# kessel/dune-pnp

Measured on AMD Instinct MI355X. Metric: assembled DOFs/s + BiCGStab iters/s, 3-species PNP on pore.msh-refined, higher is better.
Workload: dtype f64; 1 GPU; config 3: stationary 3-ion PNP, test/pore_pnp/pore.msh refined k=4 x 1 mirrored copies; dofs=2214099, dofs_per_gpu=2214099, mesh_vertices=738033, triangles=1470464, parallelism=mesh partition (RCB) x1, preconditioner=ilu0, colors=4, sell_slots=5176768, blocks=5155025

## Files before the change

### dune-pnp_amd/csrc/assemble.hip

```cpp
#include <cstdlib>

#include <hip/hip_ext.h>

#include "element.h"
#include "kernels.h"

namespace pnp {

namespace {

template <int OP, int KC = 0>
__device__ __forceinline__ void store_block(double *__restrict__ vc, int lane, int s,
                                            const double *Kc) {
  constexpr int NK = OpTraits<OP>::NK;
  static_assert(!KC || OP == OP_PNP, "constant planes: the PNP operator only");
  constexpr int Q0 = KC ? 2 : 0;
#ifdef ASM_STORE_PLAIN
  store_vals<NK, Q0>(vc + size_t(s) * NK * kRows, lane, Kc);
#else
  store_vals_nt<NK, Q0>(vc + size_t(s) * NK * kRows, lane, Kc);
#endif
}

template <int OP, int JAC, int MINW, int FANR>
__global__ __launch_bounds__(256, MINW) void k_assemble(DevLayout L, AsmArgs a) {
  using T = OpTraits<OP>;
  constexpr int NF = T::NF, NK = T::NK;
  const int row = xcd_block(blockIdx.x, gridDim.x, L.xcd_remap) * blockDim.x + threadIdx.x;
  if (row >= L.n_owned) return;
  const int chunk = row / kRows, lane = row % kRows;
  const int off = L.chunk_off[chunk];
  const uint64_t meta = L.rowmeta[row];
  const int len = int(meta & 63);
  const bool closed = (meta >> 6) & 1;
  const unsigned brk = unsigned(meta >> 8);
  const int *__restrict__ cix = L.colidx + off + lane;
  double *__restrict__ vc = a.vals + size_t(off) * NK;

  const double2 pi2 = reinterpret_cast<const double2 *>(L.xy)[row];
  double ui[NF];
#pragma unroll
  for (int f = 0; f < NF; f++) ui[f] = a.x[size_t(row) * NF + f];
  double ai = 0, aq = 0;
  if constexpr (OP == OP_DIFF || OP == OP_DIFF_IE || OP == OP_POISSON) ai = a.aux0[row];
  if constexpr (OP == OP_POISSON) aq = a.aux1[row];
  if constexpr (OP == OP_PB) pb_fifth(ui[0], ai, aq);

  double R[NF], D[NK], P[NK], F[NK];
#pragma unroll
  for (int f = 0; f < NF; f++) R[f] = 0;
#pragma unroll
  for (int v = 0; v < NK; v++) D[v] = P[v] = F[v] = 0;

  auto next_slot = [&](int s) { return (s + 1 < len) ? s + 1 : (closed ? 1 : -1); };
  auto load_nb = [&](int j, double2 &p, double (&u)[NF], double &a0, double &a1) {
    p = reinterpret_cast<const double2 *>(L.xy)[j];
    load_nf<NF>(a.x, size_t(j), u);
    if constexpr (OP == OP_DIFF || OP == OP_DIFF_IE || OP == OP_POISSON) a0 = a.aux0[j];
    if constexpr (OP == OP_POISSON) a1 = a.aux1[j];
  };
  double2 pc, pn;
  double uc[NF], un[NF];
  double ac0 = 0, ac1 = 0, an0 = 0, an1 = 0;
  constexpr int NC = FANR > 0 ? FANR : 1;
  int cj[NC];
  if constexpr (FANR > 0) {
#pragma unroll
    for (int k = 1; k < FANR; k++) cj[k] = cix[(k < len ? k : 0) * kRows];
  }
  auto col = [&](int k) -> int {
    if constexpr (FANR > 0)
      return cj[k];
    else
      return cix[k * kRows];
  };
  load_nb(col(1), pc, uc, ac0, ac1);
  if constexpr (OP == OP_PB) pb_fifth(uc[0], ac0, ac1);
  {
    const int t1 = next_slot(1);
    if (t1 > 0) load_nb(t1 == 1 ? col(1) : col(2), pn, un, an0, an1);
  }
  int jn = -1;
  if constexpr (FANR == 0) {
    const int t2 = next_slot(1) > 0 ? next_slot(next_slot(1)) : -1;
    if (t2 > 0 && next_slot(1) != 1) jn = cix[t2 * kRows];
  }
  for (int s = 1; s < len; ++s) {
    const int t = next_slot(s);
    const int tn = (t > 0 && t != 1) ? next_slot(t) : -1;
    double2 pp = pn;
    double up[NF];
    double ap0 = 0, ap1 = 0;
    if (tn > 0) {
      if constexpr (FANR > 0) {
        load_nb(tn == 1 ? col(1) : col(s + 2), pp, up, ap0, ap1);
      } else {
        load_nb(jn, pp, up, ap0, ap1);
        const int tnn = tn != 1 ? next_slot(tn) : -1;
        jn = tnn > 0 ? cix[tnn * kRows] : -1;
      }
    }
    const bool elem = t > 0 && !((brk >> s) & 1);
    if constexpr (OP == OP_PB)
      if (t > 0) pb_fifth(un[0], an0, an1);
    if (elem) {
      Geo G;
      geometry(pi2.x, pi2.y, pc.x, pc.y, pn.x, pn.y, G);
      double Ct[NK];
#pragma unroll
      for (int v = 0; v < NK; v++) Ct[v] = 0;
      element<OP, JAC>(a, G, pi2.y, pc.y, pn.y, ui, uc, un, ai, ac0, an0, aq, ac1, an1, R, D, P,
                       Ct);
      if constexpr (JAC) {
        if (s == 1 && closed) {
#pragma unroll
          for (int v = 0; v < NK; v++) F[v] = P[v];
        } else {
          store_block<OP>(vc, lane, s, P);
        }
#pragma unroll
        for (int v = 0; v < NK; v++) P[v] = Ct[v];
      }
    } else if constexpr (JAC) {
      store_block<OP>(vc, lane, s, P);
#pragma unroll
      for (int v = 0; v < NK; v++) P[v] = 0;
    }
    pc = pn;
#pragma unroll
    for (int f = 0; f < NF; f++) uc[f] = un[f];
    ac0 = an0;
    ac1 = an1;
    if (tn > 0) {
      pn = pp;
#pragma unroll
      for (int f = 0; f < NF; f++) un[f] = up[f];
      an0 = ap0;
      an1 = ap1;
    }
  }
  if constexpr (JAC) {
    if (closed) {
#pragma unroll
      for (int v = 0; v < NK; v++) F[v] += P[v];
      store_block<OP>(vc, lane, 1, F);
    }
    store_block<OP>(vc, lane, 0, D);
  }
#pragma unroll
  for (int f = 0; f < NF; f++) {
    const size_t q = size_t(row) * NF + f;
    const double rv = R[f] + a.cvec[q];
    a.r[q] = a.dmask[q] != 0 ? 0.0 : rv;
  }
}

#ifndef ASM_SU
#define ASM_SU 4
#endif
template <int OP>
__host__ __device__ constexpr int asm_lds_rec() {
  return 2 + OpTraits<OP>::NF + (OP == OP_DIFF || OP == OP_DIFF_IE || OP == OP_POISSON) +
         (OP == OP_POISSON);
}
template <int OP>
constexpr int asm_kc() {
  return OP == OP_PNP;
}
template <int OP, int JAC, int MINW, int FANR, int SPLIT = FANR, int STAGE = 0, int LDSG = 0,
          int KC = 0>
__global__ __launch_bounds__(256, MINW) void k_assemble_ga(DevLayout L, AsmArgs a) {
  using T = OpTraits<OP>;
  constexpr int NF = T::NF, NK = T::NK, NS = FANR;
  constexpr bool AUX0 = OP == OP_DIFF || OP == OP_DIFF_IE || OP == OP_POISSON;
  constexpr bool AUX1 = OP == OP_POISSON;
  constexpr int RW = asm_lds_rec<OP>();
  extern __shared__ double srec[];
  const int blk = row_block(L, blockIdx.x, gridDim.x);
  const int row0 = blk * blockDim.x + threadIdx.x;
  const bool live = row0 < L.n_owned;
  if (!LDSG && !live) return;
  const int row = live ? row0 : 0;
  const int chunk = row / kRows, lane = row % kRows;
  const int off = L.chunk_off[chunk];
  const uint64_t meta = L.rowmeta[row];
  const int len = int(meta & 63);
  const bool closed = (meta >> 6) & 1;
  const unsigned brk = unsigned(meta >> 8);
  double *__restrict__ vc = a.vals + size_t(off) * NK;

  int cj[NS];
  if constexpr (LDSG) {
    const uint16_t *__restrict__ lix = L.lidx + off + lane;
#pragma unroll
    for (int k = 1; k < NS; k++) {
      const int t = lix[(k < len ? k : 0) * kRows];
      cj[k] = k < len ? t : 0;
    }
  } else {
    const int *__restrict__ cix = L.colidx + off + lane;
#pragma unroll
    for (int k = 1; k < NS; k++) cj[k] = cix[(k < len ? k : 0) * kRows];
  }
  const double2 pi2 = reinterpret_cast<const double2 *>(L.xy)[row];
  double ui[NF];
  load_nf<NF>(a.x, size_t(row), ui);
  double ai = 0, aq = 0;
  if constexpr (AUX0) ai = a.aux0[row];
  if constexpr (AUX1) aq = a.aux1[row];
  if constexpr (OP == OP_PB) pb_fifth(ui[0], ai, aq);
  if constexpr (LDSG) {
    const int u0 = L.uptr[blk], cnt = L.uown[blk];
    constexpr int kSU = ASM_SU;
    int jj[kSU];
#pragma unroll
    for (int u = 0; u < kSU; u++) {
      const int k = int(threadIdx.x) + u * 256;
      jj[u] = k < cnt ? L.ulist[u0 + k] : -1;
    }
    double t[kSU][RW];
#pragma unroll
    for (int u = 0; u < kSU; u++)
      if (jj[u] >= 0) {
        const double2 p = reinterpret_cast<const double2 *>(L.xy)[jj[u]];
        t[u][0] = p.x;
        t[u][1] = p.y;
        double uu[NF];
        load_nf<NF>(a.x, size_t(jj[u]), uu);
#pragma unroll
        for (int f = 0; f < NF; f++) t[u][2 + f] = uu[f];
        if constexpr (AUX0) t[u][2 + NF] = a.aux0[jj[u]];
        if constexpr (AUX1) t[u][3 + NF] = a.aux1[jj[u]];
      }
#pragma unroll
    for (int u = 0; u < kSU; u++)
      if (jj[u] >= 0)
#pragma unroll
        for (int w = 0; w < RW; w++) srec[size_t(int(threadIdx.x) + u * 256) * RW + w] = t[u][w];
    for (int k = int(threadIdx.x) + kSU * 256; k < cnt; k += blockDim.x) {
      const int j = L.ulist[u0 + k];
      const double2 p = reinterpret_cast<const double2 *>(L.xy)[j];
      double u[NF];
      load_nf<NF>(a.x, size_t(j), u);
      double *r = srec + size_t(k) * RW;
      r[0] = p.x;
      r[1] = p.y;
#pragma unroll
      for (int f = 0; f < NF; f++) r[2 + f] = u[f];
      if constexpr (AUX0) r[2 + NF] = a.aux0[j];
      if constexpr (AUX1) r[3 + NF] = a.aux1[j];
    }
    __syncthreads();
    if (!live) return;
  }
  double2 pn[NS];
  double un[NS][NF], a0[NS], a1[NS];
  auto gather = [&](int k) {
    if constexpr (LDSG) {
      const double *r = srec + size_t(cj[k]) * RW;
      pn[k] = make_double2(r[0], r[1]);
#pragma unroll
      for (int f = 0; f < NF; f++) un[k][f] = r[2 + f];
      a0[k] = AUX0 ? r[2 + NF] : 0.0;
      a1[k] = AUX1 ? r[3 + NF] : 0.0;
    } else {
      pn[k] = reinterpret_cast<const double2 *>(L.xy)[cj[k]];
      load_nf<NF>(a.x, size_t(cj[k]), un[k]);
      a0[k] = AUX0 ? a.aux0[cj[k]] : 0.0;
      a1[k] = AUX1 ? a.aux1[cj[k]] : 0.0;
    }
  };
#pragma unroll
  for (int k = 1; k < SPLIT; k++) gather(k);
  if constexpr (OP == OP_PB) pb_fifth(un[1][0], a0[1], a1[1]);

  double R[NF], D[NK], P[NK], F[NK];
#pragma unroll
  for (int f = 0; f < NF; f++) R[f] = 0;
#pragma unroll
  for (int v = 0; v < NK; v++) D[v] = P[v] = F[v] = 0;
  constexpr int NSTG = (STAGE && JAC && SPLIT < NS && SPLIT > 3) ? SPLIT - 3 : 0;
  __shared__ double stg[NSTG > 0 ? NSTG * NK * 256 : 1];
  unsigned staged = 0;
  auto put = [&](int s, const double *Kc) {
    if (NSTG > 0 && s <= NSTG) {
#pragma unroll
      for (int v = 0; v < NK; v++) stg[((s - 1) * NK + v) * 256 + threadIdx.x] = Kc[v];
      staged |= 1u << s;
    } else {
      store_block<OP, KC>(vc, lane, s, Kc);
    }
  };
#pragma unroll
  for (int s = 1; s < NS; s++) {
    if (SPLIT < NS && s == (SPLIT > 2 ? SPLIT - 2 : 1)) {
#pragma unroll
      for (int k = SPLIT; k < NS; k++) gather(k);
      if constexpr (NSTG > 0) {
#pragma unroll
        for (int q = 1; q <= NSTG; q++)
          if ((staged >> q) & 1) {
            double K[NK];
#pragma unroll
            for (int v = 0; v < NK; v++) K[v] = stg[((q - 1) * NK + v) * 256 + threadIdx.x];
            store_block<OP, KC>(vc, lane, q, K);
          }
      }
    }
    if (s < len) {
      const bool has_next = s + 1 < len;
      const int sn = (s + 1 < NS) ? s + 1 : 1;
      const bool elem = (has_next || closed) && !((brk >> s) & 1);
      if constexpr (OP == OP_PB)
        if (has_next) pb_fifth(un[sn][0], a0[sn], a1[sn]);
      if (elem) {
        const double2 pt = has_next ? pn[sn] : pn[1];
        double ut[NF];
#pragma unroll
        for (int f = 0; f < NF; f++) ut[f] = has_next ? un[sn][f] : un[1][f];
        const double at0 = has_next ? a0[sn] : a0[1], at1 = has_next ? a1[sn] : a1[1];
        Geo G;
        geometry(pi2.x, pi2.y, pn[s].x, pn[s].y, pt.x, pt.y, G);
        double Ct[NK];
#pragma unroll
        for (int v = 0; v < NK; v++) Ct[v] = 0;
        element<OP, JAC, KC>(a, G, pi2.y, pn[s].y, pt.y, ui, un[s], ut, ai, a0[s], at0, aq,
                             a1[s], at1, R, D, P, Ct);
        if constexpr (JAC) {
          if (s == 1 && closed) {
#pragma unroll
            for (int v = 0; v < NK; v++) F[v] = P[v];
          } else {
            put(s, P);
          }
#pragma unroll
          for (int v = 0; v < NK; v++) P[v] = Ct[v];
        }
      } else if constexpr (JAC) {
        put(s, P);
#pragma unroll
        for (int v = 0; v < NK; v++) P[v] = 0;
      }
    }
  }
  if constexpr (JAC) {
    if (closed) {
#pragma unroll
      for (int v = 0; v < NK; v++) F[v] += P[v];
      store_block<OP, KC>(vc, lane, 1, F);
    }
    store_block<OP, KC>(vc, lane, 0, D);
  }
#pragma unroll
  for (int f = 0; f < NF; f++) {
    const size_t q = size_t(row) * NF + f;
    const double rv = R[f] + a.cvec[q];
    a.r[q] = a.dmask[q] != 0 ? 0.0 : rv;
  }
}

template <int OP>
__global__ __launch_bounds__(256) void k_mass_apply(DevLayout L, double tau, double pi, int cyl,
                                                    const double *__restrict__ xo,
                                                    double *__restrict__ cvec) {
  constexpr int NF = OpTraits<OP>::NF;
  const int row = blockIdx.x * blockDim.x + threadIdx.x;
  if (row >= L.n_owned) return;
  const int chunk = row / kRows, lane = row % kRows;
  const int off = L.chunk_off[chunk];
  const uint64_t meta = L.rowmeta[row];
  const int len = int(meta & 63);
  const bool closed = (meta >> 6) & 1;
  const int *cix = L.colidx + off + lane;
  const double2 pi2 = reinterpret_cast<const double2 *>(L.xy)[row];
  double acc = 0;
  for (int s = 1; s < len; ++s) {
    const int t = (s + 1 < len) ? s + 1 : (closed ? 1 : -1);
    if (t < 0 || ((meta >> (8 + s)) & 1)) continue;
    const int b = cix[s * kRows], c = cix[t * kRows];
    const double2 pb2 = reinterpret_cast<const double2 *>(L.xy)[b];
    const double2 pc2 = reinterpret_cast<const double2 *>(L.xy)[c];
    Geo G;
    geometry(pi2.x, pi2.y, pb2.x, pb2.y, pc2.x, pc2.y, G);
    if constexpr (OP == OP_PNP_IE) {
      double Mii, Mib, Mic;
      mass_q2(G, cyl, pi, pi2.y, pb2.y, pc2.y, Mii, Mib, Mic);
      acc += tau * ((xo[size_t(row) * 3 + 1] + xo[size_t(row) * 3 + 2]) * Mii +
                    (xo[size_t(b) * 3 + 1] + xo[size_t(b) * 3 + 2]) * Mib +
                    (xo[size_t(c) * 3 + 1] + xo[size_t(c) * 3 + 2]) * Mic);
    } else {
      acc += xo[row] * G.adet * (1.0 / 12.0) + (xo[b] + xo[c]) * G.adet * (1.0 / 24.0);
    }
  }
  if constexpr (OP == OP_PNP_IE)
    cvec[size_t(row) * NF + 1] -= acc;
  else
    cvec[row] -= acc;
}

__global__ __launch_bounds__(256) void k_ion_flux(int ns, const int4 *__restrict__ seg,
                                                  const double *__restrict__ xy,
                                                  const double *__restrict__ x, int cyl,
                                                  double pi, double *__restrict__ out) {
  const int k = blockIdx.x * blockDim.x + threadIdx.x;
  if (k >= ns) return;
  const int4 q = seg[k];
  const double2 pa = reinterpret_cast<const double2 *>(xy)[q.x];
  const double2 pc = reinterpret_cast<const double2 *>(xy)[q.y];
  const double2 po = reinterpret_cast<const double2 *>(xy)[q.z];
  Geo G;
  geometry(pa.x, pa.y, pc.x, pc.y, po.x, po.y, G);
  double gf[3][2];
#pragma unroll
  for (int f = 0; f < 3; f++) {
    const double ua = x[size_t(q.x) * 3 + f], uc = x[size_t(q.y) * 3 + f],
                 uo = x[size_t(q.z) * 3 + f];
    gf[f][0] = ua * G.gi0 + uc * G.gb0 + uo * G.gc0;
    gf[f][1] = ua * G.gi1 + uc * G.gb1 + uo * G.gc1;
  }
  const double cp = 0.5 * (x[size_t(q.x) * 3 + 1] + x[size_t(q.y) * 3 + 1]);
  const double cm = 0.5 * (x[size_t(q.x) * 3 + 2] + x[size_t(q.y) * 3 + 2]);
  const double tx = pc.x - pa.x, ty = pc.y - pa.y;
  const double len = sqrt(tx * tx + ty * ty);
  double factor = len;
  if (cyl) factor *= 2 * pi * (0.5 * (pa.y + pc.y));
  double nx = ty / len, ny = -tx / len;
  if (nx * (po.x - pa.x) + ny * (po.y - pa.y) > 0) {
    nx = -nx;
    ny = -ny;
  }
  const double gp0 = factor * gf[0][0] * cp, gp1 = factor * gf[0][1] * cp;
  out[2 * size_t(k)] = (-factor * gf[1][0] + gp0) * nx + (-factor * gf[1][1] + gp1) * ny;
  const double r = cm / cp;
  out[2 * size_t(k) + 1] =
      (-factor * gf[2][0] - gp0 * r) * nx + (-factor * gf[2][1] - gp1 * r) * ny;
}

}

hipError_t launch_ion_flux(int ns, const int4 *seg, const double *xy, const double *x, int cyl,
                           double pi, double *out, hipStream_t s) {
  if (ns == 0) return hipSuccess;
  hipLaunchKernelGGL(k_ion_flux, dim3((ns + 255) / 256), dim3(256), 0, s, ns, seg, xy, x, cyl, pi,
                     out);
  return hipGetLastError();
}

hipError_t launch_assemble(const DevLayout &L, const AsmArgs &a, hipStream_t s, hipEvent_t t0,
                           hipEvent_t t1) {
  if (L.n_owned == 0) return hipSuccess;
  dim3 grid((L.n_owned + 255) / 256), block(256);
  static const int waves = [] {
    const char *e = getenv("PNP_ASM_WAVES");
    return (e && atoi(e) == 4) ? 4 : 3;
  }();
  static const bool fanr_ok = [] {
    const char *e = getenv("PNP_ASM_FANR");
    return !(e && atoi(e) == 0);
  }();
  static const int ga = [] {
    const char *e = getenv("PNP_ASM_GA");
    return e ? atoi(e) : 4;
  }();
  const int fanr = !fanr_ok ? 0 : (L.max_slots <= 9 ? 9 : (L.max_slots <= 12 ? 12 : 0));
  static const int lds_env = [] {
    const char *e = getenv("PNP_ASM_LDS");
    return e ? (atoi(e) == 1 ? 1 : 0) : -1;
  }();
  static const bool cold_hint = [] {
    const char *e = getenv("PNP_ASM_COLD_HINT");
    return !(e && e[0] == '0');
  }();
  const auto lds_walk = [&](int nk) {
    return lds_env == 1 ||
           (lds_env < 0 && (size_t(L.n_owned) * 7 * size_t(nk) * 8 > (size_t(512) << 20) ||
                            (cold_hint && a.cold)));
  };
#define PNP_ASM_CASE(OPK)                                                          \
  case OPK:                                                                        \
    if (!fanr && a.jac)                                                            \
      hipExtLaunchKernelGGL((k_assemble<OPK, 1, 3, 0>), grid, block, 0, s, t0, t1, 0, L, a);     \
    else if (!fanr)                                                                \
      hipExtLaunchKernelGGL((k_assemble<OPK, 0, 4, 0>), grid, block, 0, s, t0, t1, 0, L, a);     \
    else if (!a.jac && fanr == 9 && ga && lds_env == 1 && L.uown &&                 \
             size_t(L.unmax) * asm_lds_rec<OPK>() * 8 <= 53 * 1024)                    \
      hipExtLaunchKernelGGL((k_assemble_ga<OPK, 0, 3, 9, 9, 0, 1>), grid, block,         \
                         size_t(L.unmax) * asm_lds_rec<OPK>() * 8, s, t0, t1, 0, L, a);             \
    else if (!a.jac && fanr == 9 && ga)                                            \
      hipExtLaunchKernelGGL((k_assemble_ga<OPK, 0, 3, 9>), grid, block, 0, s, t0, t1, 0, L, a);  \
    else if (!a.jac)                                                               \
      hipExtLaunchKernelGGL((k_assemble<OPK, 0, 4, 12>), grid, block, 0, s, t0, t1, 0, L, a);    \
    else if (ga == 1 && fanr == 9)                                                 \
      hipExtLaunchKernelGGL((k_assemble_ga<OPK, 1, 3, 9>), grid, block, 0, s, t0, t1, 0, L, a);  \
    else if (ga == 2 && fanr == 9)                                                 \
      hipExtLaunchKernelGGL((k_assemble_ga<OPK, 1, 2, 9>), grid, block, 0, s, t0, t1, 0, L, a);  \
    else if (ga == 3 && fanr == 9)                                                 \
      hipExtLaunchKernelGGL((k_assemble_ga<OPK, 1, 3, 9, 5>), grid, block, 0, s, t0, t1, 0, L, a); \
    else if (ga == 4 && fanr == 9 && asm_kc<OPK>() && a.kconst &&                   \
             lds_walk(OpTraits<OPK>::NK) && L.uown &&                               \
             size_t(L.unmax) * asm_lds_rec<OPK>() * 8 <= 53 * 1024)                    \
      hipExtLaunchKernelGGL((k_assemble_ga<OPK, 1, 3, 9, 6, 0, 1, asm_kc<OPK>()>), grid,  \
                         block, size_t(L.unmax) * asm_lds_rec<OPK>() * 8, s, t0, t1, 0, L, a); \
    else if (ga == 4 && fanr == 9 && asm_kc<OPK>() && a.kconst)                    \
      hipExtLaunchKernelGGL((k_assemble_ga<OPK, 1, 3, 9, 6, 0, 0, asm_kc<OPK>()>), grid,  \
                         block, 0, s, t0, t1, 0, L, a);                             \
    else if (ga == 4 && fanr == 9 && lds_walk(OpTraits<OPK>::NK) && L.uown &&       \
             size_t(L.unmax) * asm_lds_rec<OPK>() * 8 <= 53 * 1024)                    \
      hipExtLaunchKernelGGL((k_assemble_ga<OPK, 1, 3, 9, 6, 0, 1>), grid, block,         \
                         size_t(L.unmax) * asm_lds_rec<OPK>() * 8, s, t0, t1, 0, L, a);             \
    else if (ga == 4 && fanr == 9)                                                 \
      hipExtLaunchKernelGGL((k_assemble_ga<OPK, 1, 3, 9, 6>), grid, block, 0, s, t0, t1, 0, L, a); \
    else if (ga == 5 && fanr == 9)                                                 \
      hipExtLaunchKernelGGL((k_assemble_ga<OPK, 1, 3, 9, 3>), grid, block, 0, s, t0, t1, 0, L, a); \
    else if (ga == 6 && fanr == 9)                                                 \
      hipExtLaunchKernelGGL((k_assemble_ga<OPK, 1, 3, 9, 6, 1>), grid, block, 0, s, t0, t1, 0, L, a); \
    else if (fanr == 12)                                                           \
      hipExtLaunchKernelGGL((k_assemble<OPK, 1, 3, 12>), grid, block, 0, s, t0, t1, 0, L, a);    \
    else if (waves == 3)                                                           \
      hipExtLaunchKernelGGL((k_assemble<OPK, 1, 3, 9>), grid, block, 0, s, t0, t1, 0, L, a);     \
    else                                                                           \
      hipExtLaunchKernelGGL((k_assemble<OPK, 1, 4, 9>), grid, block, 0, s, t0, t1, 0, L, a);     \
    break;
  switch (a.kind) {
    PNP_ASM_CASE(OP_PNP)
    PNP_ASM_CASE(OP_PNP_IE)
    PNP_ASM_CASE(OP_PB)
    PNP_ASM_CASE(OP_DIFF)
    PNP_ASM_CASE(OP_DIFF_IE)
    PNP_ASM_CASE(OP_POISSON)
  default:
    return hipErrorInvalidValue;
  }
#undef PNP_ASM_CASE
  return hipGetLastError();
}

hipError_t launch_mass_apply(const DevLayout &L, int kind, double tau, double pi, int cylindrical,
                             const double *x_old, double *cvec, hipStream_t s) {
  if (L.n_owned == 0) return hipSuccess;
  dim3 grid((L.n_owned + 255) / 256), block(256);
  if (kind == OP_PNP_IE)
    hipLaunchKernelGGL(k_mass_apply<OP_PNP_IE>, grid, block, 0, s, L, tau, pi, cylindrical, x_old,
                       cvec);
  else if (kind == OP_DIFF_IE)
    hipLaunchKernelGGL(k_mass_apply<OP_DIFF_IE>, grid, block, 0, s, L, tau, pi, cylindrical,
                       x_old, cvec);
  else
    return hipErrorInvalidValue;
  return hipGetLastError();
}

}
```

### dune-pnp_amd/csrc/ctx.cc

```cpp
#include <hip/hip_runtime.h>
#include <rccl/rccl.h>
#include <rocsolver/rocsolver.h>

#include <algorithm>
#include <queue>
#include <random>
#include <chrono>
#include <condition_variable>
#include <map>
#include <unordered_map>
#include <mutex>
#include <cmath>
#include <cstdio>
#include <cstdlib>
#include <cstring>
#include <memory>
#include <string>
#include <vector>

#include "../../include/pnp_capi.h"
#include "amg.h"
#include "gmres_small.h"
#include "kernels.h"
#include "mesh.h"
// ... 73 lines not shown
  size_t h_red_n = 0;
  bool host_tr() const { return ht.exchange != nullptr; }

  int degree = 1;
  pnp::Mesh mesh, tmesh;
  pnp::PkSpace pks;
  pnp::PkDev pkd;
  DBuf<int> pk_enode, pk_ioff, pk_icnt, pk_inc;
  DBuf<uint32_t> pk_islot;
  DBuf<double> pk_eres, pk_ejac;
  DBuf<int> pk_blk_short, pk_blk_long;
  pnp::Params params;
  pnp::Fans fans;
  pnp::LocalLayout L;
  pnp::DevLayout dl;

  DBuf<int> d_chunk_len, d_chunk_off, d_colidx, d_l2g, d_send_idx, d_color_idx;
  DBuf<uint8_t> d_rowcolor;
  DBuf<uint64_t> d_rowmeta;
  DBuf<int> d_uptr, d_ulist;
  DBuf<int> d_uown;
  DBuf<int> d_lsx_ptr, d_lsx_list, d_usx_ptr, d_usx_list;
  DBuf<uint16_t> d_lsx_idx, d_usx_idx;
  DBuf<uint8_t> d_lperm, d_uperm, d_lpinv, d_upinv, d_llen, d_ulen, d_ldl;
  DBuf<uint16_t> d_lidx;
  DBuf<double> d_xy;

  int kind = -1, nf = 0, pat = 0, nvb = 0, nks = 0;
  std::vector<uint8_t> hmask;
  pnp::AsmArgs aa{};
  DBuf<double> vals, lu;
  bool lu_valid = false;
  DBuf<int> d_lchunk_len, d_lchunk_off, d_lcolidx, d_lsrc, d_uchunk_len, d_uchunk_off, d_ucolidx,
      d_usrc;
  DBuf<double> lvals, uvals, tsgs;
  int split_of = 0;
  int ilu_f32 = [] {
    const char *e = std::getenv("PNP_ILU_F32");
    const int v = e ? std::atoi(e) : 2;
    return (v >= 0 && v <= 3) ? v : 2;
  }();
  int ilu_eff() const { return (ilu_f32 >= 2 && nf == 1) ? 1 : ilu_f32; }
  int ilu_fac() const { return ilu_eff() == 3 ? 2 : ilu_eff(); }
  int f32_now() const { return split_of == 2 ? ilu_fac() : 0; }
  DBuf<float> ilu_y32buf;
  float *ilu_y32() const {
    return (split_of == 2 && ilu_eff() == 3 && !ilu_flow_opt) ? ilu_y32buf.p : nullptr;
  }
  int ilu_fused = 1;
  int amg_fallback = 0;
  int ilu_retry = 1;
  int twored_opt = [] {
    const char *ev = std::getenv("PNP_BICG_TWORED");
    return ev ? (std::atoi(ev) != 0 ? 1 : 0) : -1;
  }();
  DBuf<int> d_blkmap;
  DBuf<int> d_rowoff, d_rowcol;
  DBuf<int> d_blk_int, d_blk_bnd;
  int n_blk_int = 0, n_blk_bnd = 0;
  bool split_spmv = false;
  pnp::DevLayout sub_layout(bool interior) const {
    pnp::DevLayout d = dl;
    d.blkmap = interior ? d_blk_int.p : d_blk_bnd.p;
    const int n = interior ? n_blk_int : n_blk_bnd;
    d.blkcount = n > 0 ? n : -1;
    return d;
  }
  hipStream_t cstream = nullptr;
  hipEvent_t ev_ready = nullptr, ev_halo = nullptr;
  DBuf<double> scrub;
  bool fd_built = false, fd_mode = false;
  int fd_opt = 0;
  int fd_ne = 0;
  DBuf<int> fd_etri, fd_cdata;
  DBuf<long long> fd_rptr;
  DBuf<double> fd_jel;
  int csr_pat = -1, csr_nf = 0;
  long long csr_nnz = 0;
  DBuf<int> csr_rowptr, csr_col, csr_src;
  DBuf<unsigned char> csr_vidx;
  DBuf<double> csr_val;
  bool csr_vals_valid = false;
  struct NatDir {
    std::vector<int> lptr;
    std::vector<long long> eoff;
    DBuf<int4> info;
    DBuf<int> ecol;
    bool chain_ok = false;
    int chain_groups = 0, chain_wpad = 0;
    DBuf<int> cgptr, cecode;
    DBuf<int4> crec;
    pnp::NatFlow::Chains chains() const {
      pnp::NatFlow::Chains c;
      if (!chain_ok) return c;
      c.ngroups = chain_groups;
      c.wpad = chain_wpad;
      c.gptr = cgptr.p;
      c.rec = crec.p;
      c.ecode = cecode.p;
      return c;
    }
    pnp::NatSweep view() const {
      pnp::NatSweep w;
      w.nlev = int(lptr.size()) - 1;
      w.lptr = lptr.data();
      w.eoff = eoff.data();
      w.info = info.p;
      w.ecol = ecol.p;
      return w;
    }
  };
  NatDir nat_f, nat_b;
  DBuf<double> nat_d, nat_v, nat_vf;
  DBuf<double> nat_di, nat_vi;
  std::vector<int4> nat_units;
  DBuf<int4> d_nat_units;
  int nat_units_f = 0, nat_tail_f = 0, nat_tail_b = 0, nat_max_width = 0;
  bool nat_units_ok = false;
  DBuf<unsigned> nat_abort;
  DBuf<int> csr_diag;
  int ilu_flow_opt = [] {
    const char *e = std::getenv("PNP_ILU_FLOW");
    return (e && std::atoi(e) != 0) ? 1 : 0;
  }();
  std::vector<int> h_posrowL, h_posrowU, h_lsx_ptr, h_lsx_list, h_usx_ptr, h_usx_list;
  int64_t lslots_live = 0, uslots_live = 0;
  struct IluFlowDev {
    bool built = false, ok = false;
    pnp::IluFlow F;
    DBuf<int> dep_ptr, dep_list;
    DBuf<unsigned> flags;
  };
  IluFlowDev ilu_flow[2];
  DBuf<unsigned> ilu_flow_abort;
  bool ilu_flow_used = false;
  long long ilu_flow_n = 0;
  int seq_opt = 0;
  bool seq_built = false, seq_op_valid = false;
  DBuf<int> seq_tri, seq_vptr, seq_vinc;
  DBuf<double> seq_xy;
  std::vector<uint8_t> seq_mask_h;
  std::vector<double> seq_phi_h, seq_cp_h, seq_cm_h, seq_xold_h;
  double seq_dt = 0, seq_z = 0;
  bool seq_cextra = false;
  DBuf<unsigned char> seq_mask;
  DBuf<int> seq_bptr;
  DBuf<double> seq_bval, seq_phi, seq_cp, seq_cm, seq_xold;
  DBuf<double> seq_rl, seq_rlt, seq_rlo, seq_jl, seq_jlt, seq_vec, seq_dotv;
  int nat_pat = -1, nat_nf = 0;
  DBuf<int4> d_fseg;
  std::vector<int> fseg_group;
  DBuf<double> fluxout, fluxx, fluxred;
  DBuf<uint8_t> dmask;
  DBuf<double> cvec, aux0, aux1;
  bool assembled = false;
  bool after_solve = false;
  int mf_opt = 0;
  bool mf_lin = false, vals_stale = false;
  pnp::AsmArgs mf_aa{};
  DBuf<double> mf_x, mf_r;
  DBuf<double> mf_diag;
  DBuf<int> mf_choff;
  bool mf_diag_valid = false;
  long long mf_applies = 0, value_assemblies = 0;
  int asm_reuse_opt = [] {
    const char *e = std::getenv("PNP_ASM_REUSE_CONST");
    return (e && std::atoi(e) == 0) ? 0 : 1;
  }();
  bool vals_const_valid = false;
  long long asm_full = 0, asm_reused = 0;
  bool asm_kconst() const {
    return asm_reuse_opt && vals_const_valid && degree == 1 && !fd_mode && kind == PNP_OP_PNP;
  }
  void asm_wrote(bool kc, bool full) {
    if (kc) {
      asm_reused++;
    } else {
      asm_full++;
      vals_const_valid = full;
    }
  }

  pnp_amg_opts amg_opts{PNP_PREC_SSOR, pnp::kAmgMaxCoarse, 12, 0.8, 2, -1};
  bool amg_symmetric = true;
  std::vector<pnp::AmgLevelHost> amg_h;
  struct AmgDev {
    int nb = 0;
    DBuf<int> rp, col, dpos, mptr, mem, agg, csrc;
    DBuf<long long> cptr;
    DBuf<double> v, dinv, b, x, x2;
    DBuf<float> vf;
  };
  static bool amg_f32() {
    static const bool v = [] {
      const char *e = std::getenv("PNP_AMG_F32");
      return !(e && e[0] == '0');
    }();
    return v;
  }
  std::vector<std::unique_ptr<AmgDev>> amg_d;
  bool amg_built = false, amg_valid = false;
  int amg_nf = 0;
  double amg_setup_ms = 0;
  DBuf<double> amg_ainv, amg_x0, amg_t, amg_y, amg_r, amg_z;
  DBuf<float> amg_ainv_f;
  int amg_ld = 0;
  DBuf<int> amg_ipiv, amg_info;
  rocblas_handle blas = nullptr;


  DBuf<double> x, r, rs, z, rt, p, v, t, y, y2, b, prevu, ext, sendbuf, partials, partials2;
  DBuf<double> redmw;
  std::vector<int> newton_its;
  std::vector<double> newton_defects;
  DBuf<pnp::Scalars> S;
  pnp::Scalars *hS = nullptr;
  int gm_restart = 30;
  DBuf<double> gm_V, gm_Z, gm_part, gm_hist;
  DBuf<pnp::GmresState> gm_S;
  std::vector<double> gm_history;

  bool timing = false;
  bool debug_trace = [] {
    const char *e = std::getenv("PNP_DEBUG_BICGSTAB");
    return e && std::atoi(e) != 0;
  }();
  std::vector<std::pair<hipEvent_t, hipEvent_t>> ev_pending[T_NCAT];
  std::vector<hipEvent_t> ev_pool;
  double t_ms[T_NCAT] = {0};
  long long t_n[T_NCAT] = {0};

  ~pnp_ctx() {
    graphs_clear();
    for (auto &v : ev_pending)
      for (auto &pr : v) {
        hipEventDestroy(pr.first);
        hipEventDestroy(pr.second);
      }
    for (auto e : ev_pool) hipEventDestroy(e);
    if (hS) hipHostFree(hS);
    if (h_send) hipHostFree(h_send);
    if (h_recv) hipHostFree(h_recv);
    if (h_red) hipHostFree(h_red);
    if (comm) ncclCommDestroy(comm);
    if (blas) rocblas_destroy_handle(blas);
    if (ev_ready) hipEventDestroy(ev_ready);
    if (ev_halo) hipEventDestroy(ev_halo);
    if (cstream) hipStreamDestroy(cstream);
    if (stream) hipStreamDestroy(stream);
  }

  int graph_opt = [] {
    const char *e = std::getenv("PNP_GRAPH");
    return e ? (std::atoi(e) != 0 ? 1 : 0) : -1;
  }();
  bool use_graphs() const {
    return graph_opt == 1 || (graph_opt < 0 && L.n_owned <= (1 << 17) && !profiled());
  }
  static bool profiled() {
    static const bool p = [] {
      extern char **environ;
      for (char **e = environ; e && *e; e++)
        if (std::strncmp(*e, "ROCPROF_", 8) == 0) return true;
      return false;
    }();
    return p;
  }
  struct GraphKey {
    int count, prec, fuse, nf, pat, f32, flow;
    int mf;
    const void *zout, *dmask;
    long long epoch;
    bool operator==(const GraphKey &o) const {
      return count == o.count && prec == o.prec && fuse == o.fuse && nf == o.nf && pat == o.pat &&
             f32 == o.f32 && flow == o.flow && mf == o.mf && zout == o.zout && dmask == o.dmask &&
             epoch == o.epoch;
    }
  };
  long long graph_epoch = 0;
  bool graphs_failed = false;
  struct GraphSlot {
    GraphKey key;
    hipGraphExec_t exec = nullptr;
  };
  std::vector<GraphSlot> graph_cache;
  hipGraphExec_t nat_exec = nullptr;
  bool nat_graph_failed = false;
  void nat_graph_clear() {
    if (nat_exec) hipGraphExecDestroy(nat_exec);
    nat_exec = nullptr;
    nat_graph_failed = false;
  }
  void graphs_clear() {
    nat_graph_clear();
    for (auto &g : graph_cache)
      if (g.exec) hipGraphExecDestroy(g.exec);
    graph_cache.clear();
    graph_epoch++;
    graphs_failed = false;
  }
  template <typename F>
  int graph_run(const GraphKey &key, F &&issue, bool *captured = nullptr) {
    if (captured) *captured = true;
    for (auto &g : graph_cache)
      if (g.key == key) {
        hipError_t e = hipGraphLaunch(g.exec, stream);
        return e == hipSuccess ? PNP_OK : hipfail(e, "graph launch");
      }
    if (captured) *captured = false;
    hipError_t e = hipStreamBeginCapture(stream, hipStreamCaptureModeThreadLocal);
    if (e != hipSuccess) return hipfail(e, "graph capture");
    const int rc = issue();
    hipGraph_t graph = nullptr;
    hipError_t e2 = hipStreamEndCapture(stream, &graph);
    if (rc) {
      if (graph) hipGraphDestroy(graph);
      return rc;
    }
    if (e2 != hipSuccess) return hipfail(e2, "graph capture");
    hipGraphExec_t exec = nullptr;
    e = hipGraphInstantiate(&exec, graph, nullptr, nullptr, 0);
    hipGraphDestroy(graph);
    if (e != hipSuccess) return hipfail(e, "graph instantiate");
// ... 200 lines not shown
    if (lg) {
      std::vector<double> h(k);
      hipError_t e = hipMemcpyAsync(h.data(), d, sizeof(double) * k, hipMemcpyDeviceToHost, stream);
      if (e == hipSuccess) e = hipStreamSynchronize(stream);
      if (e != hipSuccess) return hipfail(e, "allreduce");
      lg->host[rank] = h;
      lg->barrier();
      std::vector<double> sum(k, 0.0);
      for (int r = 0; r < nranks; r++)
        for (int j = 0; j < k; j++) sum[j] += lg->host[r][j];
      lg->barrier();
      e = hipMemcpyAsync(d, sum.data(), sizeof(double) * k, hipMemcpyHostToDevice, stream);
      if (e == hipSuccess) e = hipStreamSynchronize(stream);
      return e == hipSuccess ? PNP_OK : hipfail(e, "allreduce");
    }
    if (host_tr()) {
      if (size_t(k) > h_red_n) {
        if (h_red) hipHostFree(h_red);
        h_red = nullptr;
        h_red_n = 0;
        hipError_t e = hipHostMalloc(&h_red, sizeof(double) * size_t(k));
        if (e != hipSuccess) return hipfail(e, "allreduce staging");
        h_red_n = size_t(k);
      }
      hipError_t e = hipMemcpyAsync(h_red, d, sizeof(double) * k, hipMemcpyDeviceToHost, stream);
      if (e == hipSuccess) e = hipStreamSynchronize(stream);
      if (e != hipSuccess) return hipfail(e, "allreduce");
      if (ht.allreduce_sum(ht.user, h_red, k) != 0)
        return fail(PNP_E_RCCL, "host transport: allreduce failed");
      e = hipMemcpyAsync(d, h_red, sizeof(double) * k, hipMemcpyHostToDevice, stream);
      if (e == hipSuccess) e = hipStreamSynchronize(stream);
      return e == hipSuccess ? PNP_OK : hipfail(e, "allreduce");
    }
    ncclResult_t nr = ncclAllReduce(d, d, k, ncclDouble, ncclSum, comm, stream);
    if (nr != ncclSuccess)
      return fail(PNP_E_RCCL, std::string("ncclAllReduce: ") + ncclGetErrorString(nr));
    return PNP_OK;
  }

  int allreduce_red(int k) {
    if (!dist) return PNP_OK;
    hipEvent_t t0 = tb(T_ALLRED);
    double *red = reinterpret_cast<double *>(reinterpret_cast<char *>(S.p) +
                                             offsetof(pnp::Scalars, red));
    int rc = allreduce_dev(red, k);
    if (rc) return rc;
    te(T_ALLRED, t0);
    return PNP_OK;
  }

  int reduce_derive(int np, int k, int stage, bool from2 = false) {
    hipError_t e;
    const double *src = from2 ? partials2.p : partials.p;
    if (!dist) {
      e = pnp::launch_reduce(src, np, k, S.p, stream, stage, redmw.p);
      return e == hipSuccess ? PNP_OK : hipfail(e, "reduce");
    }
    e = pnp::launch_reduce(src, np, k, S.p, stream, -1, redmw.p);
    if (e != hipSuccess) return hipfail(e, "reduce");
    int rc = allreduce_red(k);
    if (rc) return rc;
    e = pnp::launch_derive(S.p, stage, stream);
    return e == hipSuccess ? PNP_OK : hipfail(e, "derive");
  }

  int reduce_derive2(int npa, int ka, int npb, int kb, int stage) {
    hipError_t e;
    if (!dist) {
      e = pnp::launch_reduce2(partials.p, npa, ka, partials2.p, npb, kb, S.p, stream, stage,
                              redmw.p);
      return e == hipSuccess ? PNP_OK : hipfail(e, "reduce");
    }
    e = pnp::launch_reduce2(partials.p, npa, ka, partials2.p, npb, kb, S.p, stream, -1, redmw.p);
    if (e != hipSuccess) return hipfail(e, "reduce");
    int rc = allreduce_red(ka + kb);
    if (rc) return rc;
    e = pnp::launch_derive(S.p, stage, stream);
    return e == hipSuccess ? PNP_OK : hipfail(e, "derive");
  }

  int norm(const double *vec, double &out) {
    hipEvent_t t0 = tb(T_BLAS);
    hipError_t e = pnp::launch_dot(nown(), vec, vec, 0, partials.p, stream);
    if (e == hipSuccess) {
      e = pnp::launch_reduce(partials.p, pnp::blas_nparts(nown()), 1, S.p + 1, stream);
    }
    if (e != hipSuccess) return hipfail(e, "norm");
    te(T_BLAS, t0);
    if (dist) {
      double *red = reinterpret_cast<double *>(reinterpret_cast<char *>(S.p + 1) +
                                               offsetof(pnp::Scalars, red));
      int rc = allreduce_dev(red, 1);
      if (rc) return rc;
    }
    e = hipMemcpyAsync(hS + 1, S.p + 1, sizeof(pnp::Scalars), hipMemcpyDeviceToHost, stream);
    if (e == hipSuccess) e = hipStreamSynchronize(stream);
    if (e != hipSuccess) return hipfail(e, "norm readback");
    out = std::sqrt(hS[1].red[0]);
    return PNP_OK;
  }

  int upload_ext(const double *host, int nfv, double *dev, bool with_ghosts, bool devptr = false) {
    size_t ne = size_t(mesh.nv) * nfv;
    hipError_t e = hipSuccess;
    if (!devptr)
      e = hipMemcpyAsync(ext.p, host, sizeof(double) * ne, hipMemcpyHostToDevice, stream);
    if (e == hipSuccess)
      e = pnp::launch_gather_ext(with_ghosts ? L.n_owned + L.n_ghost : L.n_owned, nfv, mesh.nv,
                                 d_l2g.p, devptr ? host : ext.p, dev, stream);
    if (e != hipSuccess) return hipfail(e, "upload");
    return PNP_OK;
  }

  int download_ext(const double *dev, int nfv, double *host, bool devptr = false) {
    if (devptr) {
      hipError_t e = pnp::launch_scatter_ext(L.n_owned, nfv, mesh.nv, d_l2g.p, dev, host, stream);
      if (e == hipSuccess) e = hipStreamSynchronize(stream);
      return e == hipSuccess ? PNP_OK : hipfail(e, "download");
    }
    size_t ne = size_t(mesh.nv) * nfv;
    hipError_t e = pnp::launch_scatter_ext(L.n_owned, nfv, mesh.nv, d_l2g.p, dev, ext.p, stream);
    std::vector<double> tmp(ne);
    if (e == hipSuccess)
      e = hipMemcpyAsync(tmp.data(), ext.p, sizeof(double) * ne, hipMemcpyDeviceToHost, stream);
    if (e == hipSuccess) e = hipStreamSynchronize(stream);
    if (e != hipSuccess) return hipfail(e, "download");
    for (int i = 0; i < L.n_owned; i++) {
      int g = L.l2g[i];
      for (int f = 0; f < nfv; f++) host[size_t(f) * mesh.nv + g] = tmp[size_t(f) * mesh.nv + g];
    }
    return PNP_OK;
  }

  int assemble(const double *xdev, int jac) {
    if (kind < 0) return fail(PNP_E_STATE, "no operator set (pnp_set_operator)");
    int rc;
    if (jac && (rc = set_fd(fd_opt != 0))) return rc;
    const bool mf = jac && mf_opt && degree == 1 && !fd_mode;
    if (mf && (rc = mf_record(xdev))) return rc;
    aa.x = xdev;
    aa.jac = (fd_mode || mf) ? 0 : jac;
    aa.r = r.p;
    aa.cold = after_solve ? 1 : 0;
    aa.kconst = (aa.jac && asm_kconst()) ? 1 : 0;
    const bool one = degree == 1 && !(jac && fd_mode);
    hipEvent_t t0 = nullptr, t1 = nullptr;
    if (timing && one) {
      t0 = ev_get();
      t1 = ev_get();
    } else {
      t0 = tb(T_ASM);
    }
    hipError_t e;
    if (degree > 1)
      e = pnp::launch_pk_assemble(dl, aa, pkd, jac ? (fd_mode ? 2 : 1) : 0, stream);
    else
      e = pnp::launch_assemble(dl, aa, stream, t1 ? t0 : nullptr, t1);
    if (e == hipSuccess && jac && fd_mode && degree == 1)
      e = pnp::launch_fd_jacobian(dl, aa, nf, pat, fd_ne, fd_etri.p, fd_rptr.p, fd_cdata.p,
                                  fd_jel.p, stream);
    if (e != hipSuccess) {
      if (jac && !mf) vals_const_valid = false;
      return hipfail(e, "assemble");
    }
    if (jac && !mf) asm_wrote(aa.kconst != 0, degree == 1 && !fd_mode);
    if (t1) {
      ev_pending[T_ASM].push_back({t0, t1});
      t_n[T_ASM]++;
    } else {
      te(T_ASM, t0);
    }
    if (jac) {
      assembled = true;
      lu_valid = false;
      split_of = 0;
      amg_valid = false;
      csr_vals_valid = false;
      after_solve = false;
      mf_lin = vals_stale = mf;
      mf_diag_valid = false;
      if (!mf) value_assemblies++;
    }
    return PNP_OK;
  }

  int mf_record(const double *xdev) {
    const size_t nl = size_t(dl.n_local) * 3;
    hipError_t e = hipSuccess;
    if (mf_x.n < nl) e = mf_x.alloc(std::max<size_t>(1, nl));
    if (e == hipSuccess)
      e = hipMemcpyAsync(mf_x.p, xdev, sizeof(double) * size_t(dl.n_local) * nf,
                         hipMemcpyDeviceToDevice, stream);
    if (e != hipSuccess) return hipfail(e, "linearisation point");
    mf_aa = aa;
    mf_aa.x = mf_x.p;
    mf_aa.jac = 1;
    mf_aa.r = nullptr;
    mf_aa.cold = 0;
    return PNP_OK;
  }

  int ensure_values() {
    if (!mf_lin || !vals_stale) return PNP_OK;
    const size_t no = size_t(L.n_owned) * 3;
    hipError_t e = hipSuccess;
    if (mf_r.n < no) e = mf_r.alloc(std::max<size_t>(1, no));
    if (e != hipSuccess) return hipfail(e, "assemble at the linearisation point");
    pnp::AsmArgs fa = mf_aa;
    fa.r = mf_r.p;
    fa.vals = vals.p;
    fa.cold = after_solve ? 1 : 0;
    fa.kconst = asm_kconst() ? 1 : 0;
    hipEvent_t t0 = tb(T_ASM);
    e = pnp::launch_assemble(dl, fa, stream);
    if (e != hipSuccess) {
      vals_const_valid = false;
      return hipfail(e, "assemble at the linearisation point");
    }
    asm_wrote(fa.kconst != 0, true);
    te(T_ASM, t0);
    vals_stale = false;
    value_assemblies++;
    return PNP_OK;
  }

  int jacobi_prepare() {
    if (!mf_lin || !vals_stale || mf_diag_valid) return PNP_OK;
    hipError_t e = hipSuccess;
    if (!mf_choff.p) {
      std::vector<int> co(size_t(L.nchunks) + 1);
      for (size_t c = 0; c < co.size(); c++) co[c] = int(c) * pnp::kRows;
      int rc = upv(mf_choff, co, "diagonal layout");
      if (rc) return rc;
      e = mf_diag.alloc(std::max<size_t>(1, size_t(L.nchunks) * pnp::kRows * 6));
    }
    if (e == hipSuccess) e = pnp::launch_jac_diag(dl, mf_aa, mf_diag.p, stream);
    if (e != hipSuccess) return hipfail(e, "jacobi diagonal");
    mf_diag_valid = true;
    return PNP_OK;
  }

  int csr_structure() {
    const int nv = mesh.nv, mask = pat & 0x1FF;
    if (csr_pat == mask && csr_nf == nf) return PNP_OK;
    graphs_clear();
    const int n = nf * nv;
    std::vector<int> cnt(n + 1, 0);
    for (int i = 0; i < L.n_owned; i++) {
      const int len = pnp::meta_len(L.rowmeta[i]);
      for (int f = 0; f < nf; f++) {
        int k = 0;
        for (int g = 0; g < nf; g++) k += pnp::pat_index(mask, f, g) >= 0;
        cnt[f * nv + L.l2g[i] + 1] += k * len;
      }
    }
    for (int i = 0; i < n; i++) cnt[i + 1] += cnt[i];
    const long long nnz = cnt[n];
    std::vector<int> col(nnz), src(nnz);
    std::vector<unsigned char> vid(nnz);
    struct E {
      int col, src;
      unsigned char v;
    };
    std::vector<E> tmp;
    for (int i = 0; i < L.n_owned; i++) {
      const int chunk = i / pnp::kRows, lane = i % pnp::kRows, len = pnp::meta_len(L.rowmeta[i]);
      for (int f = 0; f < nf; f++) {
        tmp.clear();
        for (int sl = 0; sl < len; sl++) {
          const int j = L.colidx[size_t(L.chunk_off[chunk]) + size_t(sl) * pnp::kRows + lane];
          for (int g = 0; g < nf; g++) {
            const int v = pnp::pat_index(mask, f, g);
            if (v >= 0) tmp.push_back({g * nv + L.l2g[j], i << 6 | sl, (unsigned char)v});
          }
        }
        std::sort(tmp.begin(), tmp.end(), [](const E &a, const E &b) { return a.col < b.col; });
        long long q = cnt[f * nv + L.l2g[i]];
        for (const E &e : tmp) {
          col[q] = e.col;
          src[q] = e.src;
          vid[q] = e.v;
          q++;
        }
      }
    }
    int rc;
    if ((rc = upv(csr_rowptr, cnt, "csr rowptr")) || (rc = upv(csr_col, col, "csr col")) ||
        (rc = upv(csr_src, src, "csr src")) || (rc = upv(csr_vidx, vid, "csr vidx")))
      return rc;
    hipError_t e = csr_val.alloc(std::max<long long>(1, nnz));
    if (e != hipSuccess) return hipfail(e, "csr values");
    auto empty = [&](int R) { return cnt[R] == cnt[R + 1]; };
    std::vector<int> diag(n, -1);
    for (int R = 0; R < n; R++)
      for (int k = cnt[R]; k < cnt[R + 1]; k++)
        if (col[k] == R) diag[R] = k;
    for (int R = 0; R < n; R++)
      if (!empty(R) && diag[R] < 0) return fail(PNP_E_STATE, "natural SSOR: row without diagonal");
    if ((rc = upv(csr_diag, diag, "csr diagonal"))) return rc;
    auto P = [&](int R) { return L.g2l[R % nv] * nf + R / nv; };
    for (int R = 0; R < n; R++)
      if (cnt[R + 1] - cnt[R] > 255)
        return fail(PNP_E_STATE, "natural SSOR: a row has more than 255 CSR entries (row " +
                                     std::to_string(R) + ")");
    auto schedule = [&](bool fwd, NatDir &W) -> int {
      std::vector<int> &lptr = W.lptr;
      std::vector<int> lev(n, -1), push(n, 0);
      int nlev = 0;
      for (int s = 0; s < n; s++) {
        const int R = fwd ? s : n - 1 - s;
        if (empty(R)) continue;
        int l = push[R];
        for (int k = cnt[R]; k < cnt[R + 1]; k++) {
          const int C = col[k];
          if (C != R && (fwd ? C < R : C > R) && !empty(C)) l = std::max(l, lev[C] + 1);
        }
        lev[R] = l;
        nlev = std::max(nlev, l + 1);
        for (int k = cnt[R]; k < cnt[R + 1]; k++) {
          const int C = col[k];
          if (C != R && (fwd ? C > R : C < R) && !empty(C)) push[C] = std::max(push[C], l + 1);
        }
      }
      lptr.assign(nlev + 1, 0);
      for (int R = 0; R < n; R++)
        if (lev[R] >= 0) lptr[lev[R] + 1]++;
      for (int l = 0; l < nlev; l++) lptr[l + 1] += lptr[l];
      std::vector<int> fill(lptr.begin(), lptr.end() - 1), rl(std::max(1, lptr[nlev]));
      for (int R = 0; R < n; R++)
        if (lev[R] >= 0) rl[fill[lev[R]]++] = R;
      const int UR = pnp::ssor_natural_unit_rows();
      std::vector<int4> info(std::max(1, lptr[nlev]));
      std::vector<int> lwidth(nlev, 0);
      W.eoff.assign(nlev + 1, 0);
      for (int l = 0; l < nlev; l++) {
        int w = 0;
        for (int t = lptr[l]; t < lptr[l + 1]; t++) w = std::max(w, cnt[rl[t] + 1] - cnt[rl[t]]);
        lwidth[l] = w;
        W.eoff[l + 1] = W.eoff[l] + (long long)w * UR * ((lptr[l + 1] - lptr[l] + UR - 1) / UR);
      }
      std::vector<int> ecol(std::max<long long>(1, W.eoff[nlev]), -1);
      for (int l = 0; l < nlev; l++) {
        for (int t = lptr[l]; t < lptr[l + 1]; t++) {
          const int R = rl[t], len = cnt[R + 1] - cnt[R], tl = t - lptr[l];
          info[t] = make_int4(R, len | (diag[R] - cnt[R]) << 8, cnt[R], P(R));
          for (int k = 0; k < len; k++) {
            const size_t q =
                size_t(W.eoff[l]) + (size_t(tl / UR) * lwidth[l] + k) * UR + size_t(tl % UR);
            const int C = col[cnt[R] + k];
            ecol[q] = empty(C) ? -1 : fwd ? (C < R ? C : -1) : (C <= R ? C : -(C + 2));
          }
        }
      }
      static const int tail_rows = [] {
        const char *ev = std::getenv("PNP_NAT_TAIL");
        return ev ? std::max(0, std::atoi(ev)) : 0;
      }();
      static const int chain_rows = [] {
        const char *ev = std::getenv("PNP_NAT_CHAIN");
        return ev ? std::max(0, std::atoi(ev)) : std::max(0, pnp::ssor_natural_chain_capacity());
      }();
      const int trows = chain_rows > 0 ? chain_rows : tail_rows;
      int ltail = nlev;
      while (trows > 0 && ltail > 0 && lptr[ltail] - lptr[ltail - 1] <= trows) ltail--;
      W.chain_ok = false;
      if (chain_rows > 0 && ltail < nlev) {
        const int t0 = lptr[ltail], t1 = lptr[nlev];
        auto isdep = [&](int R, int C) {
          return C != R && !empty(C) && (fwd ? C < R : C > R);
        };
        std::vector<int> parent(n, -1), heavy(n, -1), hbest(n, 0);
        int wmax = 0;
// ... 2171 lines not shown
      for (int k = 0; k < 3; k++) {
        auto it = opp.find(ekey(mg.tri[3 * e + k], mg.tri[3 * e + (k + 1) % 3]));
        if (it != opp.end() && it->second < 0) it->second = mg.tri[3 * e + (k + 2) % 3];
      }
    std::vector<int4> segs;
    for (int b = 0; b < mg.nb; b++) {
      const int a = mg.bseg[2 * b], cc = mg.bseg[2 * b + 1], lo = L.g2l[std::min(a, cc)];
      if (lo < 0 || lo >= L.n_owned) continue;
      const int o = opp[ekey(a, cc)];
      const int la = L.g2l[a], lc = L.g2l[cc], lop = o >= 0 ? L.g2l[o] : -1;
      if (la < 0 || lc < 0 || lop < 0) {
        g_err = "ion flux: the element of a boundary segment is not local";
        return PNP_E_MESH;
      }
      segs.push_back(make_int4(la, lc, lop, mg.bgroup[b]));
      c->fseg_group.push_back(mg.bgroup[b]);
    }
    if ((rc = up(c->d_fseg, segs, "flux segments"))) {
      g_err = c->err;
      return rc;
    }
  }
  c->dl.lchunk_len = c->d_lchunk_len.p;
  c->dl.lchunk_off = c->d_lchunk_off.p;
  c->dl.lcolidx = c->d_lcolidx.p;
  c->dl.uchunk_len = c->d_uchunk_len.p;
  c->dl.uchunk_off = c->d_uchunk_off.p;
  c->dl.ucolidx = c->d_ucolidx.p;
  if ((rc = up(c->d_chunk_len, L.chunk_len, "chunk_len")) ||
      (rc = up(c->d_chunk_off, L.chunk_off, "chunk_off")) ||
      (rc = up(c->d_colidx, L.colidx, "colidx")) || (rc = up(c->d_rowmeta, L.rowmeta, "rowmeta")) ||
      (rc = up(c->d_xy, xy, "xy")) || (rc = up(c->d_l2g, L.l2g, "l2g")) ||
      (rc = up(c->d_send_idx, L.send_idx, "send_idx")) ||
      (rc = up(c->d_color_idx, L.color_idx, "color_idx")) ||
      (rc = up(c->d_rowcolor, L.rowcolor, "rowcolor"))) {
    g_err = c->err;
    return rc;
  }
  {
    const char *e = getenv("PNP_XCD_REMAP");
    c->dl.xcd_remap = (e && atoi(e) == 1) ? 1 : 0;
  }
  c->dl.n_owned = L.n_owned;
  c->dl.n_local = nloc;
  c->dl.nchunks = L.nchunks;
  c->dl.max_slots = L.chunk_len.empty() ? 0 : *std::max_element(L.chunk_len.begin(), L.chunk_len.end());
  c->dl.ncolors = int(L.color_ptr.size()) - 1;
  c->dl.chunk_len = c->d_chunk_len.p;
  c->dl.chunk_off = c->d_chunk_off.p;
  c->dl.colidx = c->d_colidx.p;
  c->dl.rowmeta = c->d_rowmeta.p;
  if (const char *ev = getenv("PNP_SPMV_LDS"); !(ev && atoi(ev) == 0)) {
    const int nblk = (L.n_owned + 255) / 256;
    std::vector<int> uptr(nblk + 1, 0), ulist;
    std::vector<uint16_t> lidx(size_t(L.nslots), 0);
    std::vector<int> cols, uown(nblk, 0);
    int umax = 0, unmax = 0;
    bool fits = true;
    const bool own_last = [] {
      const char *e = getenv("PNP_LIST_OWN_LAST");
      return !(e && e[0] == '0');
    }();
    for (int b = 0; b < nblk && fits; b++) {
      cols.clear();
      const int r1 = std::min(L.n_owned, 256 * b + 256);
      for (int i = 256 * b; i < r1; i++) {
        const int ch = i / pnp::kRows, ln = i % pnp::kRows;
        for (int sl = 0; sl < L.chunk_len[ch]; sl++)
          cols.push_back(L.colidx[size_t(L.chunk_off[ch]) + 64 * size_t(sl) + ln]);
      }
      std::sort(cols.begin(), cols.end());
      cols.erase(std::unique(cols.begin(), cols.end()), cols.end());
      if (cols.size() > 65535) fits = false;
      umax = std::max(umax, int(cols.size()));
      std::vector<int> npos(cols.size());
      int nn = 0;
      if (own_last) {
        std::vector<char> nb(cols.size(), 0);
        for (int i = 256 * b; i < r1; i++) {
          const int ch = i / pnp::kRows, ln = i % pnp::kRows;
          for (int sl = 1; sl < L.chunk_len[ch]; sl++) {
            const int j = L.colidx[size_t(L.chunk_off[ch]) + 64 * size_t(sl) + ln];
            if (j != i) nb[std::lower_bound(cols.begin(), cols.end(), j) - cols.begin()] = 1;
          }
        }
        for (size_t k = 0; k < cols.size(); k++)
          if (nb[k]) npos[k] = nn++;
        int no = nn;
        for (size_t k = 0; k < cols.size(); k++)
          if (!nb[k]) npos[k] = no++;
      } else {
        for (size_t k = 0; k < cols.size(); k++) npos[k] = int(k);
        nn = int(cols.size());
      }
      uown[b] = nn;
      unmax = std::max(unmax, nn);
      for (int i = 256 * b; i < r1; i++) {
        const int ch = i / pnp::kRows, ln = i % pnp::kRows;
        for (int sl = 0; sl < L.chunk_len[ch]; sl++) {
          const size_t pos = size_t(L.chunk_off[ch]) + 64 * size_t(sl) + ln;
          lidx[pos] = uint16_t(npos[std::lower_bound(cols.begin(), cols.end(), L.colidx[pos]) - cols.begin()]);
        }
      }
      std::vector<int> reord(cols.size());
      for (size_t k = 0; k < cols.size(); k++) reord[npos[k]] = cols[k];
      ulist.insert(ulist.end(), reord.begin(), reord.end());
      uptr[b + 1] = int(ulist.size());
    }
    if (fits && size_t(umax) * 3 * 8 <= 64 * 1024) {
      if ((rc = up(c->d_uptr, uptr, "uptr")) || (rc = up(c->d_ulist, ulist, "ulist")) ||
          (rc = up(c->d_lidx, lidx, "lidx")) || (rc = up(c->d_uown, uown, "uown"))) {
        g_err = c->err;
        return rc;
      }
      c->dl.uptr = c->d_uptr.p;
      c->dl.ulist = c->d_ulist.p;
      c->dl.lidx = c->d_lidx.p;
      c->dl.umax = umax;
      c->dl.uown = c->d_uown.p;
      c->dl.unmax = unmax;
    }
  }
  c->dl.xy = c->d_xy.p;
  c->dl.color_idx = c->d_color_idx.p;
  c->dl.rowcolor = c->d_rowcolor.p;
  size_t nv3 = 3 * size_t(nloc);
  auto al = [&](auto &buf, size_t n, const char *what) -> int {
    hipError_t e2 = buf.alloc(n);
    if (e2 != hipSuccess) return cp->hipfail(e2, what);
    return PNP_OK;
  };
  if ((rc = al(c->vals, size_t(L.nslots) * 8, "vals")) ||
      (rc = al(c->lu, size_t(L.nslots) * 8, "lu")) ||
      (rc = al(c->lvals, c->d_lsrc.n * 8, "lvals")) || (rc = al(c->uvals, c->d_usrc.n * 8, "uvals")) ||
      (rc = al(c->tsgs, nv3, "sgs scratch")) || (rc = al(c->fluxx, nv3, "flux state")) ||
      (rc = al(c->fluxout, 2 * c->fseg_group.size() + 2, "flux out")) ||
      (rc = al(c->fluxred, 2 * 256, "flux reduce")) || (rc = al(c->x, nv3, "x")) ||
      (rc = al(c->r, nv3, "r")) || (rc = al(c->rs, nv3, "rs")) || (rc = al(c->z, nv3, "z")) || (rc = al(c->rt, nv3, "rt")) ||
      (rc = al(c->p, nv3, "p")) || (rc = al(c->v, nv3, "v")) || (rc = al(c->t, nv3, "t")) ||
      (rc = al(c->y, nv3, "y")) || (rc = al(c->y2, nv3, "y2")) ||
      (rc = al(c->ilu_y32buf, nv3, "ILU(0) intermediate")) || (rc = al(c->b, nv3, "b")) || (rc = al(c->prevu, nv3, "prevu")) ||
      (rc = al(c->ext, 3 * size_t(c->mesh.nv), "ext")) ||
      (rc = al(c->sendbuf, 3 * std::max<size_t>(1, L.send_idx.size()), "sendbuf")) ||
      (rc = al(c->partials,
               3 * std::max<size_t>(size_t(pnp::blas_nparts(3LL * nloc)),
                                    size_t(pnp::spmv_parts(L.n_owned))) + 64,
               "partials")) ||
      (rc = al(c->partials2,
               2 * std::max<size_t>(size_t(pnp::blas_nparts(3LL * nloc)),
                                    size_t(pnp::spmv_parts(L.n_owned))) + 64,
               "partials2")) ||
      (rc = al(c->S, 2, "scalars")) || (rc = al(c->redmw, pnp::kRedMwDoubles, "reduce ticket")) ||
      (rc = al(c->dmask, 3 * size_t(L.n_owned), "dmask")) ||
      (rc = al(c->cvec, 3 * size_t(L.n_owned), "cvec")) || (rc = al(c->aux0, nloc, "aux0")) ||
      (rc = al(c->aux1, nloc, "aux1"))) {
    g_err = c->err;
    return rc;
  }
  if ((e = hipHostMalloc(&c->hS, 3 * sizeof(pnp::Scalars))) != hipSuccess) {
    g_err = std::string("hipHostMalloc: ") + hipGetErrorString(e);
    return PNP_E_HIP;
  }
  if (c->dist) {
    const char *ev = getenv("PNP_HALO_OVERLAP");
    if (!(ev && atoi(ev) == 0) && L.n_owned > 0) {
      const int nblk = (L.n_owned + 255) / 256;
      std::vector<int> order(nblk);
      if (c->d_blkmap.p) {
        CK(hipMemcpy(order.data(), c->d_blkmap.p, sizeof(int) * nblk, hipMemcpyDeviceToHost),
           "blkmap");
      } else {
        for (int b = 0; b < nblk; b++) order[b] = b;
      }
      std::vector<int> bi, bb;
      for (int b : order) {
        bool bnd = false;
        for (int i = 256 * b; i < std::min(L.n_owned, 256 * b + 256) && !bnd; i++) {
          const int ch = i / pnp::kRows, ln = i % pnp::kRows, len = pnp::meta_len(L.rowmeta[i]);
          for (int sl = 1; sl < len && !bnd; sl++)
            bnd = L.colidx[size_t(L.chunk_off[ch]) + 64 * size_t(sl) + ln] >= L.n_owned;
        }
        (bnd ? bb : bi).push_back(b);
      }
      if ((rc = up(c->d_blk_int, bi, "interior blocks")) || (rc = up(c->d_blk_bnd, bb, "boundary blocks"))) {
        g_err = c->err;
        return rc;
      }
      c->n_blk_int = int(bi.size());
      c->n_blk_bnd = int(bb.size());
      c->split_spmv = true;
      if (comm->rccl_unique_id) {
        if ((e = hipStreamCreateWithFlags(&c->cstream, hipStreamNonBlocking)) != hipSuccess ||
            (e = hipEventCreateWithFlags(&c->ev_ready, hipEventDisableTiming)) != hipSuccess ||
            (e = hipEventCreateWithFlags(&c->ev_halo, hipEventDisableTiming)) != hipSuccess) {
          g_err = std::string("halo stream: ") + hipGetErrorString(e);
          return PNP_E_HIP;
        }
      }
    }
  }
  if (degree > 1 && (rc = c->pk_build())) {
    g_err = c->err;
    return rc;
  }
  if (c->nranks > 1 && !comm->rccl_unique_id && !comm->local_group) {
    if (!comm->host->exchange || !comm->host->allreduce_sum) {
      g_err = "pnp_host_transport: exchange and allreduce_sum are required";
      return PNP_E_ARG;
    }
    c->ht = *comm->host;
    const size_t ns = 3 * std::max<size_t>(1, L.send_idx.size());
    const size_t nr = 3 * std::max<size_t>(1, size_t(L.n_ghost));
    if ((e = hipHostMalloc(&c->h_send, sizeof(double) * ns)) != hipSuccess ||
        (e = hipHostMalloc(&c->h_recv, sizeof(double) * nr)) != hipSuccess) {
      g_err = std::string("host transport staging: ") + hipGetErrorString(e);
      return PNP_E_HIP;
    }
  }
  if (c->nranks > 1 && !comm->rccl_unique_id && comm->local_group) {
    std::shared_ptr<LocalGroup> g;
    {
      std::lock_guard<std::mutex> lk(g_groups_m);
      auto &slot = g_groups[comm->local_group];
      if (!slot || slot->size != c->nranks) {
        slot = std::make_shared<LocalGroup>();
        slot->size = c->nranks;
        slot->members.assign(c->nranks, nullptr);
        slot->host.assign(c->nranks, {});
      }
      g = slot;
      if (g->members[c->rank]) {
        g_err = "rank already present in local group";
        return PNP_E_ARG;
      }
      g->members[c->rank] = c.get();
    }
    c->lg = g;
    g->barrier();
  }
  *out = c.release();
  return PNP_OK;
}

extern "C" void pnp_destroy(pnp_ctx *ctx) {
  if (!ctx) return;
  hipSetDevice(ctx->device);
  hipStreamSynchronize(ctx->stream);
  if (ctx->lg) {
    std::lock_guard<std::mutex> lk(g_groups_m);
    ctx->lg->members[ctx->rank] = nullptr;
  }
  delete ctx;
}

extern "C" int pnp_get_info(pnp_ctx *c, pnp_info *info) {
  if (!c || !info) return PNP_E_ARG;
  std::memset(info, 0, sizeof *info);
  info->nv_global = c->mesh.nv;
  info->nv_owned = c->L.n_owned;
  info->nv_ghost = c->L.n_ghost;
  info->nfields = c->nf;
  info->ncolors = int(c->L.color_ptr.size()) - 1;
  info->nchunks = c->L.nchunks;
  info->max_slots = c->fans.max_slots;
  info->nranks = c->nranks;
  info->nblocks = c->L.nblocks;
  info->nnz_reduced = c->L.nblocks * (c->nvb ? c->nvb : 1);
  info->nslots = c->L.nslots;
  info->nks = c->nks;
  info->nvb = c->nvb;
  info->lslots = (int64_t)c->d_lsrc.n;
  info->uslots = (int64_t)c->d_usrc.n;
  info->ilu_f32 = c->ilu_f32;
  info->degree = c->degree;
  info->color_conflicts = c->L.conflicts;
  info->transport = c->comm ? 2 : c->lg ? 1 : c->host_tr() ? 3 : 0;
  info->nat_flow_applies = c->nat_flow_n;
  info->nat_level_applies = c->nat_level_n;
  info->ilu_flow_applies = c->ilu_flow_n;
  info->lslots_live = c->lslots_live;
  info->uslots_live = c->uslots_live;
  info->lsx_entries = (int64_t)c->h_lsx_list.size();
  info->usx_entries = (int64_t)c->h_usx_list.size();
  size_t b = 0;
  b += c->vals.n * 8 + (c->x.n + c->r.n + c->rs.n + c->z.n + c->rt.n + c->p.n + c->v.n + c->t.n + c->y.n +
                        c->y2.n + c->b.n + c->prevu.n + c->ext.n) * 8 + c->ilu_y32buf.n * 4;
  b += c->d_colidx.n * 4 + c->d_rowmeta.n * 8 + c->d_xy.n * 8;
  b += (c->mf_x.n + c->mf_r.n + c->mf_diag.n) * 8 + c->mf_choff.n * 4;
  info->device_bytes = int64_t(b);
  return PNP_OK;
}

extern "C" int pnp_nfields(pnp_ctx *c) { return c ? c->nf : PNP_E_ARG; }

extern "C" int pnp_set_operator(pnp_ctx *c, const pnp_op_args *a) {
  if (!c || !a) return PNP_E_ARG;
  if (a->kind < PNP_OP_PNP || a->kind > PNP_OP_POISSON)
    return c->fail(PNP_E_ARG, "unknown operator kind");
  hipSetDevice(c->device);
  int kind = a->kind;
  const bool ie = kind == PNP_OP_PNP_IMPLICIT_EULER || kind == PNP_OP_DIFF_IMPLICIT_EULER;
  if (ie && !(a->dt > 0)) return c->fail(PNP_E_ARG, "implicit Euler needs dt > 0");
  if (ie && !a->x_old) return c->fail(PNP_E_ARG, "implicit Euler needs x_old");
  if ((kind == PNP_OP_DIFF || kind == PNP_OP_DIFF_IMPLICIT_EULER) &&
      (!a->phi || (a->field != 1 && a->field != 2)))
    return c->fail(PNP_E_ARG, "diffusion operator needs phi and field 1 or 2");
  if (kind == PNP_OP_POISSON && (!a->cp || !a->cm))
    return c->fail(PNP_E_ARG, "Poisson operator needs cp and cm");
  if (c->degree > 1 && (kind == PNP_OP_PNP || kind == PNP_OP_PNP_IMPLICIT_EULER))
    return c->fail(PNP_E_ARG,
                   "PnpOperator / PnpTOperator are P1 in the reference (Pk2DLocalFiniteElementMap<..., 1>, "
                   "src/stationary_pnp_from_pb.hh:206-208); P_k contexts take PB, Poisson and diffusion");
  c->kind = kind;
  c->fd_mode = false;
  c->nf = (kind == PNP_OP_PNP || kind == PNP_OP_PNP_IMPLICIT_EULER) ? 3 : 1;
  c->pat = kind == PNP_OP_PNP ? pnp::kPatPnp
                              : (kind == PNP_OP_PNP_IMPLICIT_EULER ? pnp::kPatPnpIE : pnp::kPatScalar);
  c->nvb = pnp::popc9(c->pat);
  c->nks = pnp::nks_of(c->pat);
  c->assembled = false;
  c->lu_valid = false;
  c->split_of = 0;
  c->amg_valid = false;
  c->csr_vals_valid = false;
  c->mf_lin = c->vals_stale = c->mf_diag_valid = false;
  if (c->mf_opt) c->graphs_clear();
  c->vals_const_valid = false;
  CK(hipMemsetAsync(c->vals.p, 0, sizeof(double) * size_t(c->L.nslots) * c->nks, c->stream),
     "clear matrix");
  const pnp::Mesh &m = c->mesh;
  const pnp::LocalLayout &L = c->L;
  int nf = c->nf;
  int field0 = (kind == PNP_OP_DIFF || kind == PNP_OP_DIFF_IMPLICIT_EULER) ? a->field : 0;
  std::vector<uint8_t> mask;
  if (c->degree > 1)
    pnp::pk_dirichlet_mask(c->tmesh, c->pks, c->params, nf, field0, mask);
  else
    pnp::dirichlet_mask(m, c->params, nf, field0, mask);
  std::vector<double> load(size_t(m.nv) * nf, 0.0);
  if (kind == PNP_OP_PNP || kind == PNP_OP_PNP_IMPLICIT_EULER || kind == PNP_OP_PB ||
      kind == PNP_OP_POISSON) {
    if (c->degree > 1)
      pnp::pk_neumann_load(c->tmesh, c->pks, c->params, nf, 0, load);
    else
      pnp::neumann_load(m, c->params, nf, 0, load);
    if (kind == PNP_OP_PNP_IMPLICIT_EULER)
      for (auto &v : load) v *= a->dt;
  }
  std::vector<uint8_t> lmask(size_t(L.n_owned) * nf);
  std::vector<double> lload(size_t(L.n_owned) * nf);
  for (int i = 0; i < L.n_owned; i++)
    for (int f = 0; f < nf; f++) {
      lmask[size_t(i) * nf + f] = mask[size_t(L.l2g[i]) * nf + f];
      lload[size_t(i) * nf + f] = load[size_t(L.l2g[i]) * nf + f];
      if (a->c_extra) lload[size_t(i) * nf + f] += a->c_extra[size_t(f) * m.nv + L.l2g[i]];
    }
  CK(hipMemcpy(c->dmask.p, lmask.data(), lmask.size(), hipMemcpyHostToDevice), "dmask");
  c->seq_op_valid = false;
  c->seq_dt = a->dt;
  c->seq_z = a->z;
  c->seq_cextra = a->c_extra != nullptr;
  c->seq_mask_h.assign(size_t(nf) * m.nv, 0);
  if (c->degree == 1)
    for (int g = 0; g < m.nv; g++)
      for (int f = 0; f < nf; f++) c->seq_mask_h[size_t(f) * m.nv + g] = mask[size_t(g) * nf + f];
  auto hcopy = [&](const double *h, size_t cnt, std::vector<double> &out) {
    if (h) out.assign(h, h + cnt); else out.clear();
  };
  const bool dk = kind == PNP_OP_DIFF || kind == PNP_OP_DIFF_IMPLICIT_EULER;
  hcopy(dk ? a->phi : nullptr, m.nv, c->seq_phi_h);
  hcopy(kind == PNP_OP_POISSON ? a->cp : nullptr, m.nv, c->seq_cp_h);
  hcopy(kind == PNP_OP_POISSON ? a->cm : nullptr, m.nv, c->seq_cm_h);
  hcopy(ie ? a->x_old : nullptr, size_t(nf) * m.nv, c->seq_xold_h);
  c->dl.dmask = c->dmask.p;
  c->hmask = lmask;
  CK(hipMemcpy(c->cvec.p, lload.data(), sizeof(double) * lload.size(), hipMemcpyHostToDevice),
     "cvec");
  int nloc = L.n_owned + L.n_ghost;
  auto up_field = [&](const double *h, double *d) -> int {
    std::vector<double> tmp(nloc);
    for (int i = 0; i < nloc; i++) tmp[i] = h[L.l2g[i]];
    hipError_t e = hipMemcpy(d, tmp.data(), sizeof(double) * nloc, hipMemcpyHostToDevice);
    return e == hipSuccess ? PNP_OK : c->hipfail(e, "aux upload");
  };
  int rc;
  if (kind == PNP_OP_DIFF || kind == PNP_OP_DIFF_IMPLICIT_EULER)
    if ((rc = up_field(a->phi, c->aux0.p))) return rc;
  if (kind == PNP_OP_POISSON)
    if ((rc = up_field(a->cp, c->aux0.p)) || (rc = up_field(a->cm, c->aux1.p))) return rc;
  if (ie) {
    if ((rc = c->upload_ext(a->x_old, nf, c->prevu.p, true))) return rc;
    int k = kind == PNP_OP_PNP_IMPLICIT_EULER ? pnp::OP_PNP_IE : pnp::OP_DIFF_IE;
    if (c->degree > 1)
      CK(pnp::launch_pk_mass_apply(c->dl, c->pkd, c->prevu.p, c->cvec.p, c->stream), "mass apply");
    else
      CK(pnp::launch_mass_apply(c->dl, k, c->params.tau, c->params.pi, c->params.cylindrical,
                                c->prevu.p, c->cvec.p, c->stream),
         "mass apply");
    CK(hipStreamSynchronize(c->stream), "mass apply");
  }
  pnp::AsmArgs &aa = c->aa;
  aa = pnp::AsmArgs{};
  aa.kind = kind;
  aa.l_b = c->params.l_b;
  aa.c0 = c->params.c0;
  aa.tau = c->params.tau;
  aa.pi = c->params.pi;
  aa.dt = a->dt;
  aa.z = a->z;
  aa.cylindrical = c->params.cylindrical;
  aa.aux0 = c->aux0.p;
  aa.aux1 = c->aux1.p;
  aa.cvec = c->cvec.p;
  aa.dmask = c->dmask.p;
  aa.vals = c->vals.p;
  return PNP_OK;
}

static int seq_residual_abi(pnp_ctx *c, const double *x, double *r, bool dev) {
  int rc;
  if ((rc = c->seq_build())) return rc;
  const size_t n = c->nseq();
  double *sx = c->sq(pnp_ctx::SQ_X), *sr = c->sq(pnp_ctx::SQ_R);
  CK(hipMemcpyAsync(sx, x, 8 * n, dev ? hipMemcpyDeviceToDevice : hipMemcpyHostToDevice, c->stream),
     "seq upload");
  if ((rc = c->seq_residual(sx, sr))) return rc;
  CK(hipMemcpyAsync(r, sr, 8 * n, dev ? hipMemcpyDeviceToDevice : hipMemcpyDeviceToHost, c->stream),
     "seq download");
  CK(hipStreamSynchronize(c->stream), "seq residual");
  return PNP_OK;
}
static int seq_jacobian_abi(pnp_ctx *c, const double *x, bool dev, bool fd) {
  int rc;
  if ((rc = c->seq_build())) return rc;
  double *sx = c->sq(pnp_ctx::SQ_X);
  CK(hipMemcpyAsync(sx, x, 8 * size_t(c->nseq()),
                    dev ? hipMemcpyDeviceToDevice : hipMemcpyHostToDevice, c->stream),
     "seq upload");
  if ((rc = c->seq_jacobian(sx, fd))) return rc;
  CK(hipStreamSynchronize(c->stream), "seq jacobian");
  return PNP_OK;
}

extern "C" int pnp_residual(pnp_ctx *c, const double *x, double *r) {
  if (!c || !x || !r) return PNP_E_ARG;
  if (c->kind < 0) return c->fail(PNP_E_STATE, "no operator set");
  hipSetDevice(c->device);
  if (c->seq_on()) return seq_residual_abi(c, x, r, false);
  int rc;
  if ((rc = c->upload_ext(x, c->nf, c->x.p, true))) return rc;
  if ((rc = c->assemble(c->x.p, 0))) return rc;
  return c->download_ext(c->r.p, c->nf, r);
}

extern "C" int pnp_jacobian(pnp_ctx *c, const double *x) {
  if (!c || !x) return PNP_E_ARG;
  if (c->kind < 0) return c->fail(PNP_E_STATE, "no operator set");
  hipSetDevice(c->device);
  if (c->seq_on()) return seq_jacobian_abi(c, x, false, c->fd_opt != 0);
  int rc;
  if ((rc = c->upload_ext(x, c->nf, c->x.p, true))) return rc;
  if ((rc = c->assemble(c->x.p, 1))) return rc;
  CK(hipStreamSynchronize(c->stream), "jacobian");
  return PNP_OK;
}

extern "C" int pnp_jacobian_export(pnp_ctx *c, int64_t *nnz, int32_t *rowptr, int32_t *col,
                                   double *val) {
  if (!c || !nnz) return PNP_E_ARG;
  if (!c->assembled) return c->fail(PNP_E_STATE, "no Jacobian assembled");
  if (c->seq_on()) {
    *nnz = c->csr_nnz;
    if (!rowptr || !col || !val) return PNP_OK;
    const size_t n = c->nseq();
    CK(hipMemcpy(rowptr, c->csr_rowptr.p, 4 * (n + 1), hipMemcpyDeviceToHost), "export");
    CK(hipMemcpy(col, c->csr_col.p, 4 * size_t(c->csr_nnz), hipMemcpyDeviceToHost), "export");
    CK(hipMemcpy(val, c->csr_val.p, 8 * size_t(c->csr_nnz), hipMemcpyDeviceToHost), "export");
    return PNP_OK;
  }
  const pnp::LocalLayout &L = c->L;
  int nf = c->nf, NV = c->nvb, nv = c->mesh.nv;
  long long total = 0;
  for (int i = 0; i < L.n_owned; i++) total += (long long)pnp::meta_len(L.rowmeta[i]);
  total *= NV;
  *nnz = total;
  if (!rowptr || !col || !val) return PNP_OK;
  hipSetDevice(c->device);
  if (int rc = c->ensure_values()) return rc;
  CK(hipStreamSynchronize(c->stream), "export");
  const int NKS = c->nks;
  std::vector<double> hv(size_t(L.nslots) * NKS);
  CK(hipMemcpy(hv.data(), c->vals.p, sizeof(double) * hv.size(), hipMemcpyDeviceToHost), "export");
  int n = nf * nv;
  std::vector<int> cnt(n + 1, 0);
  for (int i = 0; i < L.n_owned; i++) {
    int len = pnp::meta_len(L.rowmeta[i]);
    for (int f = 0; f < nf; f++) {
      int k = 0;
      for (int g = 0; g < nf; g++) k += pnp::pat_index(c->pat, f, g) >= 0;
      cnt[f * nv + L.l2g[i] + 1] += k * len;
    }
  }
  for (int i = 0; i < n; i++) cnt[i + 1] += cnt[i];
  std::vector<int> fill(n, 0);
  std::vector<std::pair<int, double>> tmp;
  for (int i = 0; i < L.n_owned; i++) {
    int chunk = i / pnp::kRows, lane = i % pnp::kRows;
    int len = pnp::meta_len(L.rowmeta[i]);
    for (int f = 0; f < nf; f++) {
      int R = f * nv + L.l2g[i];
      tmp.clear();
      unsigned dm = 0;
      for (int g = 0; g < nf; g++) dm |= unsigned(c->hmask[size_t(i) * nf + g] != 0) << g;
      for (int s = 0; s < len; s++) {
        int j = L.colidx[size_t(L.chunk_off[chunk]) + size_t(s) * pnp::kRows + lane];
        double K[9], B[9];
        for (int q = 0; q < NKS; q++)
          K[q] = hv[(size_t(L.chunk_off[chunk]) + size_t(s) * pnp::kRows) * NKS +
                    pnp::vin(NKS, q, lane)];
        expand_host(c->pat, K, dm, s == 0, B);
        for (int g = 0; g < nf; g++) {
          int v = pnp::pat_index(c->pat, f, g);
          if (v < 0) continue;
          tmp.push_back({g * nv + L.l2g[j], B[v]});
        }
      }
      std::sort(tmp.begin(), tmp.end());
      for (auto &pr : tmp) {
        col[cnt[R] + fill[R]] = pr.first;
        val[cnt[R] + fill[R]] = pr.second;
        fill[R]++;
      }
    }
  }
  for (int i = 0; i <= n; i++) rowptr[i] = cnt[i];
  return PNP_OK;
}

static int check_flags(pnp_ctx *c, int32_t flags, int32_t allowed) {
  if (flags & ~allowed) return c->fail(PNP_E_ARG, "unsupported flags for this call");
  return PNP_OK;
}

extern "C" int pnp_residual_ex(pnp_ctx *c, const double *x, double *r, int32_t flags) {
  if (!c || !x || !r) return PNP_E_ARG;
  if (c->kind < 0) return c->fail(PNP_E_STATE, "no operator set");
  int rc;
  if ((rc = check_flags(c, flags, PNP_DEVICE_PTRS))) return rc;
  hipSetDevice(c->device);
  const bool dev = flags & PNP_DEVICE_PTRS;
  if (c->seq_on()) return seq_residual_abi(c, x, r, dev);
  if ((rc = c->upload_ext(x, c->nf, c->x.p, true, dev))) return rc;
  if ((rc = c->assemble(c->x.p, 0))) return rc;
  return c->download_ext(c->r.p, c->nf, r, dev);
}

extern "C" int pnp_jacobian_ex(pnp_ctx *c, const double *x, int32_t flags) {
  if (!c || !x) return PNP_E_ARG;
  if (c->kind < 0) return c->fail(PNP_E_STATE, "no operator set");
  int rc;
  if ((rc = check_flags(c, flags, PNP_DEVICE_PTRS | PNP_JAC_FD))) return rc;
  hipSetDevice(c->device);
  if (c->seq_on())
    return seq_jacobian_abi(c, x, flags & PNP_DEVICE_PTRS, c->fd_opt || (flags & PNP_JAC_FD));
  if ((rc = c->upload_ext(x, c->nf, c->x.p, true, flags & PNP_DEVICE_PTRS))) return rc;
  const int keep = c->fd_opt;
  if (flags & PNP_JAC_FD) c->fd_opt = 1;
// ... 161 lines not shown
    c->amg_fallback = int(value);
    return PNP_OK;
  }
  if (option == PNP_OPT_ILU_RETRY) {
    if (value != 0 && value != 1) return c->fail(PNP_E_ARG, "PNP_OPT_ILU_RETRY takes 0 or 1");
    c->ilu_retry = int(value);
    return PNP_OK;
  }
  if (option == PNP_OPT_GMRES_RESTART) {
    if (!pnp::gm_restart_valid(value))
      return c->fail(PNP_E_ARG, "PNP_OPT_GMRES_RESTART takes 2 .. 128");
    if (c->gm_restart != int(value)) {
      hipSetDevice(c->device);
      c->gmres_free();
      c->gm_restart = int(value);
    }
    return PNP_OK;
  }
  if (option == PNP_OPT_BICG_TWORED) {
    if (value < -1 || value > 1) return c->fail(PNP_E_ARG, "PNP_OPT_BICG_TWORED takes -1, 0 or 1");
    c->twored_opt = int(value);
    return PNP_OK;
  }
  if (option == PNP_OPT_SEQ_ORDER) {
    if (value != 0 && value != 1) return c->fail(PNP_E_ARG, "PNP_OPT_SEQ_ORDER takes 0 or 1");
    if (value && (c->degree > 1 || c->dist))
      return c->fail(PNP_E_ARG, "PNP_OPT_SEQ_ORDER: P1 contexts of one rank only");
    if (c->seq_opt != int(value)) {
      c->seq_opt = int(value);
      c->assembled = false;
      c->csr_vals_valid = false;
      c->mf_lin = c->vals_stale = c->mf_diag_valid = false;
    }
    return PNP_OK;
  }
  if (option == PNP_OPT_MATRIX_FREE) {
    if (value != 0 && value != 1) return c->fail(PNP_E_ARG, "PNP_OPT_MATRIX_FREE takes 0 or 1");
    if (value && c->degree > 1)
      return c->fail(PNP_E_STATE,
                     "PNP_OPT_MATRIX_FREE: P1 contexts only (the matrix-free application walks the "
                     "P1 vertex fans; P_k contexts assemble)");
    if (!value && c->mf_lin) {
      hipSetDevice(c->device);
      if (int rc = c->ensure_values()) return rc;
      c->mf_lin = c->mf_diag_valid = false;
    }
    c->mf_opt = int(value);
    return PNP_OK;
  }
  if (option == PNP_OPT_ASM_REUSE_CONST) {
    if (value != 0 && value != 1)
      return c->fail(PNP_E_ARG, "PNP_OPT_ASM_REUSE_CONST takes 0 or 1");
    c->asm_reuse_opt = int(value);
    return PNP_OK;
  }
  if (option == PNP_OPT_JAC_FD) {
    if (value != 0 && value != 1) return c->fail(PNP_E_ARG, "PNP_OPT_JAC_FD takes 0 or 1");
    c->fd_opt = int(value);
    return PNP_OK;
  }
  if (option == PNP_OPT_ILU_FUSED_FACTOR) {
    if (value != 0 && value != 1) return c->fail(PNP_E_ARG, "PNP_OPT_ILU_FUSED_FACTOR takes 0 or 1");
    c->ilu_fused = int(value);
    c->lu_valid = false;
    if (c->split_of == 2) c->split_of = 0;
    return PNP_OK;
  }
  return c->fail(PNP_E_ARG, "unknown option");
}

extern "C" int pnp_set_create_option(int32_t option, int64_t value) {
  if (option == PNP_CREATE_ABSORB_THIN_COLOR) {
    if (value < -1 || value > 1) {
      g_err = "PNP_CREATE_ABSORB_THIN_COLOR takes -1, 0 or 1";
      return PNP_E_ARG;
    }
    pnp::g_absorb_thin_color.store(int(value));
    return PNP_OK;
  }
  g_err = "unknown creation option";
  return PNP_E_ARG;
}

extern "C" int pnp_get_create_option(int32_t option, int64_t *value) {
  if (!value) return PNP_E_ARG;
  if (option == PNP_CREATE_ABSORB_THIN_COLOR) {
    *value = pnp::g_absorb_thin_color.load();
    return PNP_OK;
  }
  g_err = "unknown creation option";
  return PNP_E_ARG;
}

extern "C" int pnp_get_option(pnp_ctx *c, int32_t option, int64_t *value) {
  if (!c || !value) return PNP_E_ARG;
  if (option == PNP_OPT_ILU_F32) {
    *value = c->ilu_f32;
    return PNP_OK;
  }
  if (option == PNP_OPT_ILU_FUSED_FACTOR) {
    *value = c->ilu_fused;
    return PNP_OK;
  }
  if (option == PNP_OPT_GRAPH) {
    *value = c->graph_opt;
    return PNP_OK;
  }
  if (option == PNP_OPT_JAC_FD) {
    *value = c->fd_opt;
    return PNP_OK;
  }
  if (option == PNP_OPT_GMRES_RESTART) {
    *value = c->gm_restart;
    return PNP_OK;
  }
  if (option == PNP_OPT_BICG_TWORED) {
    *value = c->twored_opt;
    return PNP_OK;
  }
  if (option == PNP_OPT_ILU_FLOW) {
    *value = c->ilu_flow_opt;
    return PNP_OK;
  }
  if (option == PNP_OPT_AMG_FALLBACK) {
    *value = c->amg_fallback;
    return PNP_OK;
  }
  if (option == PNP_OPT_ILU_RETRY) {
    *value = c->ilu_retry;
    return PNP_OK;
  }
  if (option == PNP_OPT_SEQ_ORDER) {
    *value = c->seq_opt;
    return PNP_OK;
  }
  if (option == PNP_OPT_MATRIX_FREE) {
    *value = c->mf_opt;
    return PNP_OK;
  }
  if (option == PNP_OPT_ASM_REUSE_CONST) {
    *value = c->asm_reuse_opt;
    return PNP_OK;
  }
  return c->fail(PNP_E_ARG, "unknown option");
}

extern "C" int pnp_matfree_info(pnp_ctx *c, int64_t *applies, int64_t *value_assemblies) {
  if (!c) return PNP_E_ARG;
  if (applies) *applies = c->mf_applies;
  if (value_assemblies) *value_assemblies = c->value_assemblies;
  return PNP_OK;
}

extern "C" int pnp_asm_info(pnp_ctx *c, int64_t *full, int64_t *reused) {
  if (!c) return PNP_E_ARG;
  if (full) *full = c->asm_full;
  if (reused) *reused = c->asm_reused;
  return PNP_OK;
}

extern "C" int pnp_amg_configure(pnp_ctx *c, const pnp_amg_opts *o) {
  if (!c || !o) return PNP_E_ARG;
  if (o->smoother != PNP_PREC_SSOR && o->smoother != PNP_PREC_ILU0 &&
      o->smoother != PNP_PREC_JACOBI && o->smoother != PNP_PREC_SSOR_NATURAL)
    return c->fail(PNP_E_ARG, "AMG smoother must be SSOR, SSOR_NATURAL, ILU0 or JACOBI");
  if (o->coarse_target < 1 || o->coarse_target > pnp::kAmgMaxCoarse || o->max_levels < 2 ||
      o->max_levels > pnp::kAmgMaxLevels || !(o->omega > 0 && o->omega <= 2) ||
      o->coarse_sweeps < 1 || o->coarse_sweeps > 8 || o->level0_presmooth < -1 ||
      o->level0_presmooth > 1)
    return c->fail(PNP_E_ARG, "AMG options out of range");
  const bool rebuild = o->coarse_target != c->amg_opts.coarse_target ||
                       o->max_levels != c->amg_opts.max_levels;
  c->amg_opts = *o;
  if (rebuild) c->amg_built = false;
  c->amg_valid = false;
  return PNP_OK;
}

extern "C" int pnp_amg_info(pnp_ctx *c, pnp_amg_stats *st) {
  if (!c || !st) return PNP_E_ARG;
  std::memset(st, 0, sizeof *st);
  if (!c->amg_built) return c->fail(PNP_E_STATE, "AMG not set up (solve or apply with PNP_PREC_AMG)");
  st->levels = int(c->amg_h.size()) + 1;
  st->rows[0] = c->L.n_owned;
  st->blocks[0] = c->L.nblocks;
  for (size_t k = 0; k < c->amg_h.size() && k + 1 < 16; k++) {
    st->rows[k + 1] = c->amg_h[k].nb;
    st->blocks[k + 1] = (int64_t)c->amg_h[k].col.size();
  }
  st->omega = c->amg_opts.omega;
  st->smoother = c->amg_opts.smoother;
  return PNP_OK;
}

extern "C" int pnp_amg_aggregates(pnp_ctx *c, int32_t level, int32_t *agg) {
  if (!c || !agg || level < 0) return PNP_E_ARG;
  if (!c->amg_built) return c->fail(PNP_E_STATE, "AMG not set up");
  if (level >= int(c->amg_h.size())) return c->fail(PNP_E_ARG, "no such AMG level");
  const std::vector<int> &a = c->amg_h[level].agg;
  if (level == 0) {
    for (int g = 0; g < c->mesh.nv; g++) agg[g] = -1;
    for (int i = 0; i < c->L.n_owned; i++) agg[c->L.l2g[i]] = a[i];
  } else {
    std::copy(a.begin(), a.end(), agg);
  }
  return PNP_OK;
}

extern "C" int pnp_ion_flux(pnp_ctx *c, const double *x, int32_t nsurf, double *ip, double *im) {
  if (!c || !ip || !im || nsurf < 0 || nsurf > 256) return PNP_E_ARG;
  hipSetDevice(c->device);
  const double *xd = c->x.p;
  int rc;
  if (x) {
    if ((rc = c->upload_ext(x, 3, c->fluxx.p, true))) return rc;
    xd = c->fluxx.p;
  } else if (c->nf != 3) {
    return c->fail(PNP_E_STATE, "ion flux of the context state needs a 3-field (PNP) operator");
  }
  const int ns = int(c->fseg_group.size());
  if (c->degree > 1)
    CK(pnp::launch_pk_ion_flux(c->dl, c->pkd, ns, c->d_fseg.p, xd, c->params.cylindrical,
                               c->params.pi, c->fluxout.p, c->stream),
       "ion flux");
  else
    CK(pnp::launch_ion_flux(ns, c->d_fseg.p, c->d_xy.p, xd, c->params.cylindrical, c->params.pi,
                            c->fluxout.p, c->stream),
       "ion flux");
  std::vector<double> out(2 * size_t(ns)), acc(2 * size_t(nsurf), 0.0);
  if (ns) {
    CK(hipMemcpyAsync(out.data(), c->fluxout.p, sizeof(double) * out.size(),
                      hipMemcpyDeviceToHost, c->stream),
       "ion flux");
  }
  CK(hipStreamSynchronize(c->stream), "ion flux");
  for (int k = 0; k < ns; k++) {
    const int g = c->fseg_group[k];
    if (g < 0 || g >= nsurf) return c->fail(PNP_E_ARG, "boundary group outside [0, nsurf)");
    acc[2 * size_t(g)] += out[2 * size_t(k)];
    acc[2 * size_t(g) + 1] += out[2 * size_t(k) + 1];
  }
  if (c->dist && nsurf > 0) {
    CK(hipMemcpy(c->fluxred.p, acc.data(), sizeof(double) * acc.size(), hipMemcpyHostToDevice),
       "ion flux");
    if ((rc = c->allreduce_dev(c->fluxred.p, 2 * nsurf))) return rc;
    CK(hipStreamSynchronize(c->stream), "ion flux");
    CK(hipMemcpy(acc.data(), c->fluxred.p, sizeof(double) * acc.size(), hipMemcpyDeviceToHost),
       "ion flux");
  }
  for (int g = 0; g < nsurf; g++) {
    ip[g] = acc[2 * size_t(g)];
    im[g] = acc[2 * size_t(g) + 1];
  }
  return PNP_OK;
}

static int seq_newton(pnp_ctx *c, double *u, const pnp_newton_opts *o, pnp_newton_result *res) {
  int rc;
  if ((rc = c->seq_build())) return rc;
  double t_start = now_s();
  const size_t n = c->nseq();
  double *x = c->sq(pnp_ctx::SQ_X), *r = c->sq(pnp_ctx::SQ_R), *z = c->sq(pnp_ctx::SQ_Z),
         *prevu = c->sq(pnp_ctx::SQ_PREVU);
  CK(hipMemcpyAsync(x, u, 8 * n, hipMemcpyHostToDevice, c->stream), "seq upload");
  double ta = now_s();
  if ((rc = c->seq_residual(x, r))) return rc;
  double defect = std::sqrt(c->seq_dot(r, r, rc));
  if (rc) return rc;
  res->assemble_seconds += now_s() - ta;
  res->first_defect = defect;
  double prev_defect = defect;
  res->status = PNP_OK;
  const bool fd = c->fd_opt != 0;
  for (;;) {
    res->converged = (defect < o->abs_limit || defect < res->first_defect * o->reduction) ? 1 : 0;
    if (res->converged) break;
    if (res->iterations >= o->maxit) {
      res->status = PNP_E_NOT_CONVERGED;
      break;
    }
    ta = now_s();
    if ((rc = c->seq_jacobian(x, fd))) return rc;
    CK(hipStreamSynchronize(c->stream), "seq jacobian");
    res->assemble_seconds += now_s() - ta;
    const double stop_defect = std::max(res->first_defect * o->reduction, o->abs_limit);
    double lin_red;
    if (stop_defect / (10 * defect) > defect * defect / (prev_defect * prev_defect))
      lin_red = stop_defect / (10 * defect);
    else
      lin_red = std::min(o->min_linear_reduction, defect * defect / (prev_defect * prev_defect));
    prev_defect = defect;
    CK(hipMemsetAsync(z, 0, 8 * n, c->stream), "seq z");
    pnp_solve_opts lo = o->linear;
    lo.reduction = lin_red;
    pnp_solve_result sr{};
    double ts = now_s();
    if ((rc = c->seq_krylov(lo, z, r, sr))) return rc;
    res->solve_seconds += now_s() - ts;
    res->linear_iterations += sr.iterations;
    const int step_its = sr.iterations;
    if (sr.breakdown) {
      res->status = PNP_E_BREAKDOWN;
      break;
    }
    if (!sr.converged) {
      res->status = PNP_E_NOT_CONVERGED;
      break;
    }
    double lambda = 1.0, best_lambda = 0.0, best_defect = defect;
    CK(hipMemcpyAsync(prevu, x, 8 * n, hipMemcpyDeviceToDevice, c->stream), "seq prevu");
// ... 550 lines not shown
```

### dune-pnp_amd/csrc/kernels.h

```cpp
#pragma once

#include <hip/hip_runtime.h>

#include <cstdint>

namespace pnp {

constexpr int kRows = 64;

__device__ __forceinline__ int xcd_block(int b, int nwg, int on = 1) {
  if (!on) return b;
  const int q = nwg / 8, r = nwg % 8, xcd = b % 8;
  return (xcd < r ? xcd * (q + 1) : r * (q + 1) + (xcd - r) * q) + b / 8;
}

typedef double double2_a8 __attribute__((ext_vector_type(2), aligned(8)));
template <int NF>
__device__ __forceinline__ void load_nf(const double *__restrict__ x, size_t j, double (&o)[NF]) {
  const double *b = x + size_t(NF) * j;
  int f = 0;
#pragma unroll
  for (; f + 1 < NF; f += 2) {
    const double2_a8 a = *reinterpret_cast<const double2_a8 *>(b + f);
    o[f] = a.x;
// ... 33 lines not shown

template <int NV>
__device__ __forceinline__ void load_vals(const double *__restrict__ sb, int lane, double *B) {
#pragma unroll
  for (int q = 0; q + 1 < NV; q += 2) {
    const double2 t = reinterpret_cast<const double2 *>(sb + (q >> 1) * 2 * kRows)[lane];
    B[q] = t.x;
    B[q + 1] = t.y;
  }
  if constexpr (NV & 1) B[NV - 1] = sb[(NV - 1) * kRows + lane];
}

template <int NV>
__device__ __forceinline__ void load_vals_nt(const double *__restrict__ sb, int lane, double *B) {
#pragma unroll
  for (int q = 0; q + 1 < NV; q += 2) {
    typedef double d2v __attribute__((ext_vector_type(2)));
    const d2v t = __builtin_nontemporal_load(reinterpret_cast<const d2v *>(sb + (q >> 1) * 2 * kRows) + lane);
    B[q] = t.x;
    B[q + 1] = t.y;
  }
  if constexpr (NV & 1) B[NV - 1] = __builtin_nontemporal_load(sb + (NV - 1) * kRows + lane);
}

template <int NV, int Q0 = 0>
__device__ __forceinline__ void store_vals(double *__restrict__ sb, int lane, const double *B) {
  static_assert(Q0 % 2 == 0 && Q0 < NV, "whole 16-B records only");
#pragma unroll
  for (int q = Q0; q + 1 < NV; q += 2)
    reinterpret_cast<double2 *>(sb + (q >> 1) * 2 * kRows)[lane] = make_double2(B[q], B[q + 1]);
  if constexpr (NV & 1) sb[(NV - 1) * kRows + lane] = B[NV - 1];
}

template <int NV, int Q0 = 0>
__device__ __forceinline__ void store_vals_nt(double *__restrict__ sb, int lane, const double *B) {
  static_assert(Q0 % 2 == 0 && Q0 < NV, "whole 16-B records only");
  typedef double d2v __attribute__((ext_vector_type(2)));
#pragma unroll
  for (int q = Q0; q + 1 < NV; q += 2) {
    d2v t;
    t.x = B[q];
    t.y = B[q + 1];
    __builtin_nontemporal_store(t, reinterpret_cast<d2v *>(sb + (q >> 1) * 2 * kRows) + lane);
  }
  if constexpr (NV & 1) __builtin_nontemporal_store(B[NV - 1], sb + (NV - 1) * kRows + lane);
}

template <class DL>
__device__ __forceinline__ int row_block(const DL &L, int b, int nwg) {
  return L.blkmap ? L.blkmap[xcd_block(b, nwg, 1)] : xcd_block(b, nwg, L.xcd_remap);
}

enum OpKind : int {
  OP_PNP = 0,
  OP_PNP_IE = 1,
  OP_PB = 2,
  OP_DIFF = 3,
  OP_DIFF_IE = 4,
  OP_POISSON = 5
};

constexpr int kPatPnp = 0x1FF & ~((1 << 5) | (1 << 7));
constexpr int kPatPnpIE = 0x1FF & ~(1 << 7);
constexpr int kPatScalar = 1;
constexpr int kPatFD = 1 << 9;
constexpr int kPatPnpFD = kPatPnp | kPatFD;
constexpr int kPatPnpIEFD = kPatPnpIE | kPatFD;

__host__ __device__ constexpr int popc9(int m) {
  int c = 0;
  for (int i = 0; i < 9; i++) c += (m >> i) & 1;
  return c;
}
__host__ __device__ constexpr int pat_index(int mask, int f, int g) {
  if (!((mask >> (f * 3 + g)) & 1)) return -1;
  int c = 0;
  for (int i = 0; i < f * 3 + g; i++) c += (mask >> i) & 1;
  return c;
}

__host__ __device__ constexpr int nks_of(int pat) {
  return (pat & kPatFD) ? popc9(pat) : (pat == kPatPnp ? 5 : (pat == kPatPnpIE ? 6 : 1));
}

template <int PAT>
__host__ __device__ __forceinline__ void expand_k(const double *K, double *B) {
  if constexpr ((PAT & kPatFD) != 0) {
#pragma unroll
    for (int q = 0; q < popc9(PAT); q++) B[q] = K[q];
  } else if constexpr (PAT == kPatPnp || PAT == kPatPnpIE) {
    B[pat_index(PAT, 0, 0)] = K[0];
    B[pat_index(PAT, 0, 1)] = K[1];
    B[pat_index(PAT, 0, 2)] = -K[1];
    B[pat_index(PAT, 1, 0)] = -K[2];
    B[pat_index(PAT, 1, 1)] = K[0] - K[4];
    B[pat_index(PAT, 2, 0)] = K[3];
    B[pat_index(PAT, 2, 2)] = K[0] + K[4];
    if constexpr (PAT == kPatPnpIE) {
      B[pat_index(PAT, 1, 1)] += K[5];
      B[pat_index(PAT, 1, 2)] = K[5];
    }
  } else {
    B[0] = K[0];
  }
}

template <int NF, int PAT>
__host__ __device__ __forceinline__ void mask_rows(double *B, unsigned dm, bool diag) {
#pragma unroll
  for (int f = 0; f < NF; f++)
#pragma unroll
    for (int g = 0; g < NF; g++) {
      const int v = pat_index(PAT, f, g);
      if (v >= 0 && ((dm >> f) & 1)) B[v] = (diag && f == g) ? 1.0 : 0.0;
    }
}

struct DevLayout {
  int n_owned = 0, n_local = 0, nchunks = 0, ncolors = 0;
  int max_slots = 0;
  int xcd_remap = 0;
  const int *chunk_len = nullptr;
  const int *chunk_off = nullptr;
  const int *colidx = nullptr;
  const uint64_t *rowmeta = nullptr;
  const double *xy = nullptr;
  const int *color_idx = nullptr;
  const uint8_t *rowcolor = nullptr;
  const int *blkmap = nullptr;
  int blkcount = 0;
  const int *lchunk_len = nullptr, *lchunk_off = nullptr, *lcolidx = nullptr;
  const int *uchunk_len = nullptr, *uchunk_off = nullptr, *ucolidx = nullptr;
  const uint8_t *dmask = nullptr;
  const int *uptr = nullptr, *ulist = nullptr;
  const uint16_t *lidx = nullptr;
  int umax = 0;
  const int *uown = nullptr;
  int unmax = 0;
  const int *lsx_ptr = nullptr, *lsx_list = nullptr, *usx_ptr = nullptr, *usx_list = nullptr;
  const uint8_t *lperm = nullptr, *uperm = nullptr, *lpinv = nullptr, *upinv = nullptr;
  const uint8_t *llen = nullptr, *ulen = nullptr, *ldl = nullptr;
  const uint16_t *lsx_idx = nullptr, *usx_idx = nullptr;
  int sx_max = 0;
};

template <int NF>
__device__ __forceinline__ unsigned row_mask(const DevLayout &L, int row) {
  unsigned dm = 0;
#pragma unroll
  for (int f = 0; f < NF; f++) dm |= unsigned(L.dmask[size_t(row) * NF + f] != 0) << f;
  return dm;
}

struct AsmArgs {
  int kind;
  int jac;
  double l_b, c0, tau, pi, dt, z;
  int cylindrical;
  const double *x;
  const double *aux0;
  const double *aux1;
  const double *cvec;
  const uint8_t *dmask;
  double *r;
  double *vals;
  int cold;
  int kconst;
};

struct Scalars {
  double rho, rho_new, alpha, omega, h, norm0, norm, reduction;
  double it_half;
  double red[6];
  int done;
  int breakdown;
  int iter;
  int divguard;
  int pending;
  int xpend;
};

hipError_t launch_assemble(const DevLayout &L, const AsmArgs &a, hipStream_t s,
                           hipEvent_t t0 = nullptr, hipEvent_t t1 = nullptr);
hipError_t launch_ion_flux(int ns, const int4 *seg, const double *xy, const double *x, int cyl,
                           double pi, double *out, hipStream_t s);
hipError_t launch_mass_apply(const DevLayout &L, int kind, double tau, double pi, int cylindrical,
                             const double *x_old, double *cvec, hipStream_t s);

hipError_t launch_spmv(const DevLayout &L, int nf, int pat, const double *vals, const double *x,
                       double *y, int mode, const double *w, double *partials, int *nparts,
                       hipStream_t s, const double *w2 = nullptr, hipEvent_t t0 = nullptr,
                       hipEvent_t t1 = nullptr);

hipError_t launch_jac_apply(const DevLayout &L, const AsmArgs &a, const double *z, double *y,
                            int mode, const double *w, double *partials, int *nparts,
                            hipStream_t s, const double *w2 = nullptr, hipEvent_t t0 = nullptr,
                            hipEvent_t t1 = nullptr);
hipError_t launch_jac_diag(const DevLayout &L, const AsmArgs &a, double *dvals, hipStream_t s);

hipError_t launch_jacobi(const DevLayout &L, int nf, int pat, const double *vals, const double *d,
                         double *v, hipStream_t s);
hipError_t launch_sgs(const DevLayout &L, const int *color_ptr_host, int nf, int pat,
                      const double *lv, const double *uv, const double *d, double *v, double *t,
                      hipStream_t s);
hipError_t launch_split(const DevLayout &L, int nf, int pat, int from_k, const double *src,
                        const int *lsrc, long long ln, const int *usrc, long long un, void *lv,
                        void *uv, hipStream_t s, int f32 = 0);
hipError_t launch_expand(const DevLayout &L, int nf, int pat, const double *vals, double *lu,
                         hipStream_t s);
hipError_t launch_ilu0_factor(const DevLayout &L, const int *color_ptr_host, int nf, int pat,
                              double *lu, hipStream_t s);
hipError_t launch_ilu0_factor_fused(const DevLayout &L, const int *color_ptr_host, int nf, int pat,
                                    const double *kvals, const int *rowoff, const int *rowcol,
                                    double *aos, void *lv, void *uv, int f32, hipStream_t s);
hipError_t launch_ilu0_apply(const DevLayout &L, const int *color_ptr_host, int nf, int pat,
                             const void *lv, const void *uv, const double *d, double *v,
                             hipStream_t s, int c_first = 0, const double *add = nullptr,
                             double *out = nullptr, int f32 = 0, float *yf = nullptr,
                             hipEvent_t t0 = nullptr, hipEvent_t t1 = nullptr);
constexpr int kIluFlowMaxStages = 32;
struct IluFlow {
  int nstages = 0, nunits = 0;
  int persistent = 1;
  int unit0[kIluFlowMaxStages + 1] = {};
  int kind[kIluFlowMaxStages] = {};
  int r0[kIluFlowMaxStages] = {}, r1[kIluFlowMaxStages] = {};
  int blk0[kIluFlowMaxStages] = {};
  const int *dep_ptr = nullptr, *dep_list = nullptr;
  unsigned *flags = nullptr;
  unsigned *abort_word = nullptr;
};
hipError_t launch_ilu0_flow(const DevLayout &L, const IluFlow &F, int nf, int pat, const void *lv,
                            const void *uv, const double *d, double *v, hipStream_t s, int f32);
hipError_t launch_update_fwd0(const DevLayout &L, int nf, int pat, int c0_end, const Scalars *S,
                              int which, int first, double *x, const double *yin, double *r,
                              const double *v, double *p, const void *uv, double *yout,
                              double *partials, int *nparts, hipStream_t s, int f32 = 0,
                              const double *rt = nullptr, float *youtf = nullptr);

int blas_nparts(long long n);
hipError_t launch_update_p(long long n, const Scalars *S, const double *r, const double *v,
                           double *p, int first, hipStream_t s);
hipError_t launch_cg_update_p(long long n, const Scalars *S, const double *q, double *p,
                              hipStream_t s);
hipError_t launch_update_xr(long long n, const Scalars *S, int which, double *x, const double *y,
                            double *r, const double *v, const double *rt, double *partials,
                            hipStream_t s, const double *y1 = nullptr);
hipError_t launch_dot(long long n, const double *a, const double *b, int two, double *partials,
                      hipStream_t s);
constexpr int kRedMwDoubles = 1 + 64 * 5;
hipError_t launch_reduce(const double *partials, int nparts, int k, Scalars *S, hipStream_t s,
                         int derive_stage = -1, double *mw = nullptr);
int spmv_parts(int nrows);
hipError_t launch_reduce2(const double *pa, int npa, int ka, const double *pb, int npb, int kb,
                          Scalars *S, hipStream_t s, int derive_stage = -1, double *mw = nullptr);
hipError_t launch_derive(Scalars *S, int stage, hipStream_t s);

hipError_t launch_axpby(long long n, double a, const double *x, double b, const double *y,
                        double *out, hipStream_t s);
hipError_t launch_pack(int n, int nf, const int *idx, const double *x, double *buf, hipStream_t s);
hipError_t launch_gather_ext(int n, int nf, int nv_global, const int *l2g, const double *ext,
                             double *in, hipStream_t s);
hipError_t launch_scatter_ext(int n, int nf, int nv_global, const int *l2g, const double *in,
                              double *ext, hipStream_t s);
hipError_t launch_fd_jacobian(const DevLayout &L, const AsmArgs &aa, int nf, int pat, int ne,
                              const int *etri, const long long *rptr, const int *cdata,
                              double *jel, hipStream_t s);
hipError_t launch_csr_fill(const DevLayout &L, int nf, int pat, const double *vals, long long nnz,
                           const int *src, const unsigned char *vidx, double *out, hipStream_t s);
struct NatSweep {
  int nlev = 0;
  const int *lptr = nullptr;
  const long long *eoff = nullptr;
  const int4 *info = nullptr;
  const int *ecol = nullptr;
};
hipError_t launch_ssor_natural(const NatSweep &fwd, const NatSweep &bwd, const double *val,
                               const double *d, double *v, hipStream_t s);
int ssor_natural_unit_rows();
int ssor_natural_chain_width();
int ssor_natural_chain_history();
int ssor_natural_chain_capacity();
struct NatFlow {
  const int4 *units = nullptr;
  int nunits = 0, nunits_f = 0;
  int tail_f = 0, tail_b = 0;
  int max_width = 0;
  struct Chains {
    int ngroups = 0, wpad = 0;
    const int *gptr = nullptr, *ecode = nullptr;
    const int4 *rec = nullptr;
  } chain_f, chain_b;
  NatSweep fwd, bwd;
  unsigned *abort_word = nullptr;
};
int ssor_natural_flow_resident(const NatFlow &F, unsigned *probe, hipStream_t s);
hipError_t launch_ssor_natural_flow(const NatFlow &F, int n, const double *val, const double *d,
                                    double *vf, double *vb, hipStream_t s);
struct SeqMesh {
  int nv = 0, nt = 0;
  const int *tri = nullptr, *vptr = nullptr, *vinc = nullptr;
  const double *xy = nullptr;
};
struct SeqOp {
  int kind = 0, nf = 1, cyl = 0;
  double pi = 3.1415, l_b = 1, c0 = 0, tau = 1, dt = 0, z = 0;
  const double *phi = nullptr, *cp = nullptr, *cm = nullptr, *x_old = nullptr;
};
hipError_t launch_seq_element(const SeqMesh &M, const SeqOp &P, const double *x, int mode,
                              double *RL, double *RLT, double *RLO, double *JL, double *JLT,
                              const int *bptr, const double *bval, hipStream_t s);
hipError_t launch_seq_residual_gather(const SeqMesh &M, int nf, int has_old, const double *RL,
                                      const double *RLT, const double *RLO,
                                      const unsigned char *mask, double *r, hipStream_t s);
hipError_t launch_seq_jacobian_gather(const SeqMesh &M, int nf, const double *JL,
                                      const double *JLT, const int *rowptr, const int *col,
                                      const unsigned char *mask, double *val, hipStream_t s);
hipError_t launch_seq_spmv(int n, const int *rowptr, const int *col, const double *val,
                           const double *x, double *y, hipStream_t s);
hipError_t launch_seq_dot(int n, const double *a, const double *b, double *out, hipStream_t s);
hipError_t launch_seq_bicg_p(int n, double beta, double omega, double *p, const double *v,
                             const double *r, hipStream_t s);
hipError_t launch_seq_axpy2(int n, double a, double *x, const double *y, double *r,
                            const double *v, hipStream_t s);
hipError_t launch_seq_prec_diag(int n, int jacobi, const double *d, const int *diag,
                                const double *val, double *v, hipStream_t s);
hipError_t launch_seq_axpy(int n, double a, double *x, const double *y, hipStream_t s);
hipError_t launch_seq_aymx(int n, double a, double *x, const double *y, hipStream_t s);
hipError_t launch_seq_cg_p(int n, double beta, double *p, const double *q, hipStream_t s);

struct GmresState;
int gmres_nparts(long long n);
hipError_t launch_gmres_orth(int mode, GmresState *S, double *V, long long ld, long long n,
                             double *part, int nps, int jmax, hipStream_t s);
hipError_t launch_gmres_hess(GmresState *S, double *hist, double *V, long long ld, long long n,
                             hipStream_t s);
// ... 34 lines not shown
```

### dune-pnp_amd/python/pnp_amd/__init__.py

```python
from __future__ import annotations

import ctypes as C
import os
from dataclasses import dataclass

import numpy as np

HERE = os.path.dirname(os.path.abspath(__file__))
PKG_ROOT = os.path.dirname(os.path.dirname(HERE))
REPO_ROOT = os.path.dirname(PKG_ROOT)
LIB_PATH = os.environ.get("PNP_AMD_LIB") or os.path.join(PKG_ROOT, "libpnp_amd.so")
HEADER = os.path.join(REPO_ROOT, "include", "pnp_capi.h")

OK, E_ARG, E_HIP, E_RCCL, E_BREAKDOWN, E_NOT_CONVERGED, E_IO, E_MESH, E_STATE = \
    0, -1, -2, -3, -4, -5, -6, -7, -8
OP_PNP, OP_PNP_IMPLICIT_EULER, OP_PB, OP_DIFF, OP_DIFF_IMPLICIT_EULER, OP_POISSON = range(6)
PREC_NONE, PREC_SSOR, PREC_ILU0, PREC_JACOBI, PREC_AMG, PREC_SSOR_NATURAL = range(6)
METHOD_BICGSTAB, METHOD_CG, METHOD_GMRES, METHOD_FGMRES = 0, 1, 2, 3
(OPT_ILU_F32, OPT_ILU_FUSED_FACTOR, OPT_JAC_FD, OPT_BICG_TWORED, OPT_AMG_FALLBACK,
 OPT_GRAPH, OPT_SEQ_ORDER, OPT_ILU_FLOW, OPT_NAT_FLOW, OPT_ILU_RETRY,
 OPT_GMRES_RESTART, OPT_MATRIX_FREE, OPT_ASM_REUSE_CONST) = (1, 2, 3, 4, 5, 6, 7, 8, 9, 10, 11,
                                                             12, 13)
DEVICE_PTRS, JAC_FD = 1, 2
CREATE_ABSORB_THIN_COLOR = 1
PREC_BY_NAME = {"none": PREC_NONE, "nonprec": PREC_NONE, "ssor": PREC_SSOR, "ilu0": PREC_ILU0,
                "jacobi": PREC_JACOBI, "amg": PREC_AMG, "ssor_natural": PREC_SSOR_NATURAL}
MAX_SURFACES = 64


class PnpError(RuntimeError):
    def __init__(self, code, msg):
        super().__init__(f"pnp error {code}: {msg}")
        self.code = code


class _Mesh(C.Structure):
    _fields_ = [("nv", C.c_int32), ("coords", C.c_void_p), ("nt", C.c_int32),
                ("tri", C.c_void_p), ("nbseg", C.c_int32), ("bseg", C.c_void_p),
                ("bseg_group", C.c_void_p)]


class _Surface(C.Structure):
    _fields_ = [("coulomb_btype", C.c_int32), ("coulomb_flux", C.c_double),
                ("coulomb_potential", C.c_double), ("plus_btype", C.c_int32),
                ("plus_flux", C.c_double), ("plus_concentration", C.c_double),
                ("minus_btype", C.c_int32), ("minus_flux", C.c_double),
                ("minus_concentration", C.c_double)]


class _Params(C.Structure):
    _fields_ = [("l_b", C.c_double), ("c0", C.c_double), ("tau", C.c_double), ("pi", C.c_double),
                ("cylindrical", C.c_int32), ("n_surfaces", C.c_int32), ("surfaces", C.c_void_p)]


class _Config(C.Structure):
    _fields_ = [("meshfile", C.c_char * 1024), ("n_surfaces", C.c_int32),
                ("verbosity", C.c_int32), ("cylindrical", C.c_int32),
                ("linear_solver_iterations", C.c_int32), ("l_b", C.c_double),
                ("newton_reassemble_threshold", C.c_double), ("newton_reduction", C.c_double),
                ("newton_min_linear_reduction", C.c_double), ("newton_max_iterations", C.c_int32),
                ("newton_line_search_max_iteration", C.c_int32), ("c0", C.c_double),
                ("tau", C.c_double), ("output_freq", C.c_int32), ("n_steps", C.c_int32),
                ("potential_update_freq", C.c_int32), ("surfaces", _Surface * MAX_SURFACES),
                ("defaulted", C.c_uint32)]


_EXCHANGE_FN = C.CFUNCTYPE(C.c_int32, C.c_void_p, C.c_int32, C.POINTER(C.c_int32),
                           C.POINTER(C.c_double), C.POINTER(C.c_int64), C.POINTER(C.c_int64),
                           C.POINTER(C.c_double), C.POINTER(C.c_int64), C.POINTER(C.c_int64))
_ALLREDUCE_FN = C.CFUNCTYPE(C.c_int32, C.c_void_p, C.POINTER(C.c_double), C.c_int32)


class _HostTransport(C.Structure):
    _fields_ = [("user", C.c_void_p), ("exchange", _EXCHANGE_FN),
                ("allreduce_sum", _ALLREDUCE_FN)]


class _Comm(C.Structure):
    _fields_ = [("rank", C.c_int32), ("size", C.c_int32), ("rccl_unique_id", C.c_void_p),
                ("local_group", C.c_char_p), ("host", C.POINTER(_HostTransport))]


class TorchDistTransport:

    def __init__(self, dist=None):
        import torch
        if dist is None:
            import torch.distributed as dist
        self.dist, self.torch = dist, torch
        self.calls = {"exchange": 0, "allreduce": 0}

    def exchange(self, peers, sends, rcounts):
        self.calls["exchange"] += 1
        reqs, outs = [], []
        for q, peer in enumerate(peers):
            buf = self.torch.empty(int(rcounts[q]), dtype=self.torch.float64)
            outs.append(buf)
            if len(sends[q]):
                reqs.append(self.dist.isend(self.torch.from_numpy(sends[q]), peer))
            if rcounts[q]:
                reqs.append(self.dist.irecv(buf, peer))
        for r in reqs:
            r.wait()
        return [o.numpy() for o in outs]

    def allreduce_sum(self, buf):
        self.calls["allreduce"] += 1
        self.dist.all_reduce(self.torch.from_numpy(buf))


def _host_transport(obj):
    def exchange(_u, nq, nbr, sbuf, soff, scnt, rbuf, roff, rcnt):
        try:
            peers = [nbr[q] for q in range(nq)]
            sends = [np.ctypeslib.as_array(sbuf, shape=(max(1, soff[q] + scnt[q]),))
                     [soff[q]:soff[q] + scnt[q]].copy() for q in range(nq)]
            got = obj.exchange(peers, sends, [rcnt[q] for q in range(nq)])
            for q in range(nq):
                if rcnt[q]:
                    dst = np.ctypeslib.as_array(rbuf, shape=(roff[q] + rcnt[q],))
                    dst[roff[q]:roff[q] + rcnt[q]] = got[q]
            return 0
        except Exception:
            import traceback
            traceback.print_exc()
            return 1

    def allreduce(_u, buf, k):
        try:
            obj.allreduce_sum(np.ctypeslib.as_array(buf, shape=(k,)))
            return 0
        except Exception:
            import traceback
            traceback.print_exc()
            return 1
    fx, fa = _EXCHANGE_FN(exchange), _ALLREDUCE_FN(allreduce)
    return _HostTransport(None, fx, fa), (fx, fa)


class _Info(C.Structure):
    _fields_ = [("nv_global", C.c_int32), ("nv_owned", C.c_int32), ("nv_ghost", C.c_int32),
                ("nfields", C.c_int32), ("ncolors", C.c_int32), ("nchunks", C.c_int32),
                ("max_slots", C.c_int32), ("nranks", C.c_int32), ("nblocks", C.c_int64),
                ("nnz_reduced", C.c_int64), ("nslots", C.c_int64), ("device_bytes", C.c_int64),
                ("nks", C.c_int32), ("nvb", C.c_int32), ("lslots", C.c_int64),
                ("uslots", C.c_int64), ("ilu_f32", C.c_int32), ("degree", C.c_int32),
                ("color_conflicts", C.c_int64), ("transport", C.c_int32),
                ("nat_flow_applies", C.c_int64), ("nat_level_applies", C.c_int64),
                ("ilu_flow_applies", C.c_int64), ("lslots_live", C.c_int64),
                ("uslots_live", C.c_int64), ("lsx_entries", C.c_int64),
                ("usx_entries", C.c_int64)]


class _SpaceInfo(C.Structure):
    _fields_ = [("degree", C.c_int32), ("nnodes", C.c_int32), ("nt", C.c_int32),
                ("nlocal", C.c_int32)]


class _StoreProbe(C.Structure):
    _fields_ = [("us_sell", C.c_double), ("us_tile", C.c_double), ("us_tile_sorted", C.c_double),
                ("us_random", C.c_double),
                ("slot_bytes", C.c_int64), ("rows", C.c_int64), ("rows_whole", C.c_int64),
                ("tiles", C.c_int64), ("elements", C.c_int64)]


class _OpArgs(C.Structure):
    _fields_ = [("kind", C.c_int32), ("dt", C.c_double), ("z", C.c_double),
                ("field", C.c_int32), ("phi", C.c_void_p), ("cp", C.c_void_p),
                ("cm", C.c_void_p), ("x_old", C.c_void_p), ("c_extra", C.c_void_p)]


class _SolveOpts(C.Structure):
    _fields_ = [("prec", C.c_int32), ("reduction", C.c_double), ("maxit", C.c_int32),
                ("check_every", C.c_int32), ("method", C.c_int32)]

# ... 402 lines not shown
                                          C.c_void_p(z_ptr), C.c_void_p(y_ptr),
                                          DEVICE_PTRS | (JAC_FD if fd else 0)))

    def linear_solve_dev(self, rhs_ptr, z_ptr, prec=PREC_NONE, reduction=1e-8, maxit=20000,
                         check_every=8, method=0):
        o = _SolveOpts(prec, reduction, maxit, check_every, method)
        r = _SolveResult()
        rc = lib().pnp_linear_solve_ex(self.h, C.c_void_p(rhs_ptr), C.c_void_p(z_ptr), C.byref(o),
                                       C.byref(r), DEVICE_PTRS)
        if rc not in (OK, E_BREAKDOWN):
            self._ck(rc)
        return {k: getattr(r, k) for k, _ in _SolveResult._fields_}

    def jacobian_csr_device(self):
        v = _CsrView()
        self._ck(lib().pnp_jacobian_csr_device(self.h, C.byref(v)))
        return {"n": v.n, "nnz": v.nnz, "rowptr": v.rowptr, "col": v.col, "val": v.val}

    def linear_solve(self, rhs, prec=PREC_NONE, reduction=1e-8, maxit=20000, check_every=8,
                     method=0):
        rhs = self._vec(rhs)
        z = np.zeros_like(rhs)
        o = _SolveOpts(prec, reduction, maxit, check_every, method)
        r = _SolveResult()
        rc = lib().pnp_linear_solve(self.h, _ptr(rhs), _ptr(z), C.byref(o), C.byref(r))
        if rc not in (OK, E_BREAKDOWN):
            self._ck(rc)
        return z, {k: getattr(r, k) for k, _ in _SolveResult._fields_}

    def solve_history(self):
        n = C.c_int32(0)
        self._ck(lib().pnp_solve_history(self.h, None, 0, C.byref(n)))
        d = np.zeros(n.value)
        if n.value:
            self._ck(lib().pnp_solve_history(self.h, _ptr(d), n.value, C.byref(n)))
        return d

    def prec_apply(self, d, prec):
        d = self._vec(d)
        v = np.zeros_like(d)
        self._ck(lib().pnp_prec_apply(self.h, int(prec), _ptr(d), _ptr(v)))
        return v

    def amg_configure(self, smoother=PREC_SSOR, coarse_target=1024, max_levels=12, omega=0.8,
                      coarse_sweeps=2, level0_presmooth=-1):
        o = _AmgOpts(int(smoother), int(coarse_target), int(max_levels), float(omega),
                     int(coarse_sweeps), int(level0_presmooth))
        self._ck(lib().pnp_amg_configure(self.h, C.byref(o)))

    def amg_info(self):
        st = _AmgStats()
        self._ck(lib().pnp_amg_info(self.h, C.byref(st)))
        n = st.levels
        return {"levels": n, "rows": list(st.rows[:n]), "blocks": list(st.blocks[:n]),
                "smoother": st.smoother, "omega": st.omega}

    def amg_aggregates(self, level):
        info = self.amg_info()
        n = self.nn if level == 0 else info["rows"][level]
        agg = np.zeros(n, dtype=np.int32)
        self._ck(lib().pnp_amg_aggregates(self.h, int(level), _ptr(agg)))
        return agg

    def ion_flux(self, x=None, nsurf=None):
        n = int(nsurf if nsurf is not None else len(self.params.surfaces))
        ip = np.zeros(n)
        im = np.zeros(n)
        xv = None if x is None else np.ascontiguousarray(x, dtype=np.float64)
        if xv is not None and xv.size != 3 * self.nn:
            raise PnpError(E_ARG, "ion_flux needs a 3-field state")
        self._ck(lib().pnp_ion_flux(self.h, _ptr(xv), n, _ptr(ip), _ptr(im)))
        return ip, im

    def newton(self, u, reduction=1e-9, abs_limit=1e-12, min_linear_reduction=1e-8, maxit=50,
               line_search_maxit=500, prec=PREC_NONE, linear_maxit=20000, check_every=8,
               method=0):
        u = self._vec(u).copy()
        o = _NewtonOpts(reduction, abs_limit, min_linear_reduction, maxit, line_search_maxit,
                        _SolveOpts(prec, 0.0, linear_maxit, check_every, method))
        r = _NewtonResult()
        self._ck(lib().pnp_newton(self.h, _ptr(u), C.byref(o), C.byref(r)))
        return u, {k: getattr(r, k) for k, _ in _NewtonResult._fields_}

    def dot(self, a, b, nfields=None):
        a = np.ascontiguousarray(a, dtype=np.float64)
        b = np.ascontiguousarray(b, dtype=np.float64)
        out = C.c_double(0)
        self._ck(lib().pnp_dot(self.h, _ptr(a), _ptr(b), nfields or (a.size // self.nn), 0,
                               C.byref(out)))
        return out.value

    def norm(self, a, nfields=None):
        a = np.ascontiguousarray(a, dtype=np.float64)
        out = C.c_double(0)
        self._ck(lib().pnp_norm(self.h, _ptr(a), nfields or (a.size // self.nn), 0, C.byref(out)))
        return out.value

    def newton_history(self):
        n = C.c_int32(0)
        self._ck(lib().pnp_newton_history(self.h, None, None, 0, C.byref(n)))
        its = np.zeros(n.value, dtype=np.int32)
        dfs = np.zeros(n.value)
        self._ck(lib().pnp_newton_history(self.h, _ptr(its), _ptr(dfs), n.value, C.byref(n)))
        return its, dfs

    def sync_vector(self, v, nfields=None):
        nf = nfields or (v.size // self.nn)
        v = np.ascontiguousarray(v, dtype=np.float64).copy()
        self._ck(lib().pnp_sync_vector(self.h, _ptr(v), int(nf)))
        return v

    def initial_state(self, phi_pb):
        phi = np.ascontiguousarray(phi_pb, dtype=np.float64)
        x0 = np.zeros(3 * self.nn)
        self._ck(lib().pnp_initial_state(self.h, _ptr(phi), _ptr(x0)))
        return x0

    def state_set(self, x):
        x = self._vec(x)
        self._ck(lib().pnp_state_set(self.h, _ptr(x)))

    def state_get(self):
        x = np.zeros(self.nf * self.nn)
        self._ck(lib().pnp_state_get(self.h, _ptr(x)))
        return x

    def assemble_state(self, n=1):
        self._ck(lib().pnp_assemble_state(self.h, int(n)))

    def assemble_state_timed(self, n=1):
        ms = C.c_double()
        self._ck(lib().pnp_assemble_state_timed(self.h, int(n), C.byref(ms)))
        return ms.value / 1e3

    def bicgstab_iterations(self, n, prec=PREC_NONE):
        r = _SolveResult()
        self._ck(lib().pnp_bicgstab_iterations(self.h, int(n), int(prec), C.byref(r)))
        return {k: getattr(r, k) for k, _ in _SolveResult._fields_}

    def set_option(self, option, value):
        self._ck(lib().pnp_set_option(self.h, int(option), C.c_int64(int(value))))

    def get_option(self, option):
        v = C.c_int64()
        self._ck(lib().pnp_get_option(self.h, int(option), C.byref(v)))
        return v.value

    def matfree_info(self):
        a, v = C.c_int64(), C.c_int64()
        self._ck(lib().pnp_matfree_info(self.h, C.byref(a), C.byref(v)))
        return {"applies": a.value, "value_assemblies": v.value}

    def asm_info(self):
        f, r = C.c_int64(), C.c_int64()
        self._ck(lib().pnp_asm_info(self.h, C.byref(f), C.byref(r)))
        return {"full": f.value, "reused": r.value}

    def probe_slot_stores(self, tile_elems=256, reps=20):
        o = _StoreProbe()
        self._ck(lib().pnp_probe_slot_stores(self.h, int(tile_elems), int(reps), C.byref(o)))
        return {k: getattr(o, k) for k, _ in _StoreProbe._fields_}

    def cache_scrub(self, nbytes=1 << 30):
        self._ck(lib().pnp_cache_scrub(self.h, C.c_int64(int(nbytes))))

    def timers(self, enable=None, reset=False):
        if enable is not None:
            self._ck(lib().pnp_timers_enable(self.h, int(bool(enable))))
        if reset:
            self._ck(lib().pnp_timers_reset(self.h))
        t = _Timers()
        self._ck(lib().pnp_timers_get(self.h, C.byref(t)))
        return {k: getattr(t, k) for k, _ in _Timers._fields_}


def header_symbols():
    import re
    txt = open(HEADER).read()
    return sorted(set(re.findall(r"^\s*(?:int|void|const char \*)\s*(pnp_\w+)\s*\(", txt, re.M)))


def header_constants():
    import re
    txt = open(HEADER).read()
    return {k: int(v) for k, v in re.findall(r"^\s*(PNP_\w+)\s*=\s*(-?\d+)\s*,?\s*$", txt, re.M)}
```

### include/pnp_capi.h

```cpp
#ifndef PNP_CAPI_H
#define PNP_CAPI_H

#include <stdint.h>

#ifdef __cplusplus
extern "C" {
#endif

#define PNP_CAPI_VERSION 1

enum {
  PNP_OK = 0,
  PNP_E_ARG = -1,
  PNP_E_HIP = -2,
  PNP_E_RCCL = -3,
  PNP_E_BREAKDOWN = -4,
  PNP_E_NOT_CONVERGED = -5,
  PNP_E_IO = -6,
  PNP_E_MESH = -7,
  PNP_E_STATE = -8
};

typedef struct pnp_ctx pnp_ctx;

// ... 45 lines not shown
  uint32_t defaulted;
} pnp_config;

int pnp_config_read(const char *path, pnp_config *out);

typedef struct {
  void *user;
  int32_t (*exchange)(void *user, int32_t nnbr, const int32_t *nbr, const double *sbuf,
                      const int64_t *soff, const int64_t *scount, double *rbuf,
                      const int64_t *roff, const int64_t *rcount);
  int32_t (*allreduce_sum)(void *user, double *buf, int32_t k);
} pnp_host_transport;

typedef struct {
  int32_t rank, size;
  const void *rccl_unique_id;
  const char *local_group;
  const pnp_host_transport *host;
} pnp_comm;

int pnp_create(const pnp_mesh *mesh, const pnp_params *params, int32_t device,
               const pnp_comm *comm, pnp_ctx **out);
int pnp_create_pk(const pnp_mesh *mesh, const pnp_params *params, int32_t degree, int32_t device,
                  const pnp_comm *comm, pnp_ctx **out);
void pnp_destroy(pnp_ctx *ctx);
const char *pnp_last_error(const pnp_ctx *ctx);
int pnp_rccl_unique_id(void *out128);

typedef struct {
  int32_t nv_global, nv_owned, nv_ghost, nfields;
  int32_t ncolors, nchunks, max_slots, nranks;
  int64_t nblocks;
  int64_t nnz_reduced;
  int64_t nslots;
  int64_t device_bytes;
  int32_t nks;
  int32_t nvb;
  int64_t lslots, uslots;
  int32_t ilu_f32;
  int32_t degree;
  int64_t color_conflicts;
  int32_t transport;
  int64_t nat_flow_applies;
  int64_t nat_level_applies;
  int64_t ilu_flow_applies;
  int64_t lslots_live, uslots_live;
  int64_t lsx_entries, usx_entries;
} pnp_info;
int pnp_get_info(pnp_ctx *ctx, pnp_info *info);

typedef struct {
  int32_t degree, nnodes, nt, nlocal;
} pnp_space_info;
int pnp_space(pnp_ctx *ctx, pnp_space_info *info, double *xy, int32_t *enode);

enum {
  PNP_OP_PNP = 0,
  PNP_OP_PNP_IMPLICIT_EULER,
  PNP_OP_PB,
  PNP_OP_DIFF,
  PNP_OP_DIFF_IMPLICIT_EULER,
  PNP_OP_POISSON
};

typedef struct {
  int32_t kind;
  double dt;
  double z;
  int32_t field;
  const double *phi;
  const double *cp, *cm;
  const double *x_old;
  const double *c_extra;
} pnp_op_args;

int pnp_set_operator(pnp_ctx *ctx, const pnp_op_args *args);
int pnp_nfields(pnp_ctx *ctx);

int pnp_residual(pnp_ctx *ctx, const double *x, double *r);
int pnp_jacobian(pnp_ctx *ctx, const double *x);
int pnp_jacobian_export(pnp_ctx *ctx, int64_t *nnz, int32_t *rowptr, int32_t *col, double *val);

enum {
  PNP_DEVICE_PTRS = 1,
  PNP_JAC_FD = 2
};
int pnp_residual_ex(pnp_ctx *ctx, const double *x, double *r, int32_t flags);
int pnp_jacobian_ex(pnp_ctx *ctx, const double *x, int32_t flags);
int pnp_jacobian_apply(pnp_ctx *ctx, const double *x, const double *z, double *y, int32_t flags);
typedef struct {
  int32_t n;
  int64_t nnz;
  const int32_t *rowptr;
  const int32_t *col;
  const double *val;
} pnp_csr_view;
int pnp_jacobian_csr_device(pnp_ctx *ctx, pnp_csr_view *view);

enum { PNP_PREC_NONE = 0, PNP_PREC_SSOR = 1, PNP_PREC_ILU0 = 2, PNP_PREC_JACOBI = 3,
       PNP_PREC_AMG = 4,
       PNP_PREC_SSOR_NATURAL = 5 };
enum { PNP_METHOD_BICGSTAB = 0, PNP_METHOD_CG = 1,
       PNP_METHOD_GMRES = 2,
       PNP_METHOD_FGMRES = 3 };
typedef struct {
  int32_t prec;
  double reduction;
  int32_t maxit;
  int32_t check_every;
  int32_t method;
} pnp_solve_opts;
typedef struct {
  int32_t converged, iterations, breakdown;
  double it_half, defect0, defect, reduction, elapsed;
} pnp_solve_result;

int pnp_prec_apply(pnp_ctx *ctx, int32_t prec, const double *d, double *v);

typedef struct {
  int32_t smoother;
  int32_t coarse_target;
  int32_t max_levels;
  double omega;
  int32_t coarse_sweeps;
  int32_t level0_presmooth;
} pnp_amg_opts;
int pnp_amg_configure(pnp_ctx *ctx, const pnp_amg_opts *opts);
typedef struct {
  int32_t levels;
  int32_t smoother;
  int32_t rows[16];
  int64_t blocks[16];
  double omega;
} pnp_amg_stats;
int pnp_amg_info(pnp_ctx *ctx, pnp_amg_stats *stats);
int pnp_amg_aggregates(pnp_ctx *ctx, int32_t level, int32_t *agg);

enum {
  PNP_OPT_ILU_F32 = 1,
  PNP_OPT_ILU_FUSED_FACTOR = 2,
  PNP_OPT_JAC_FD = 3,
  PNP_OPT_BICG_TWORED = 4,
  PNP_OPT_AMG_FALLBACK = 5,
  PNP_OPT_GRAPH = 6,
  PNP_OPT_SEQ_ORDER = 7,
  PNP_OPT_ILU_FLOW = 8,
  PNP_OPT_NAT_FLOW = 9,
  PNP_OPT_ILU_RETRY = 10,
  PNP_OPT_GMRES_RESTART = 11,
  PNP_OPT_MATRIX_FREE = 12,
  PNP_OPT_ASM_REUSE_CONST = 13
};
int pnp_set_option(pnp_ctx *ctx, int32_t option, int64_t value);
int pnp_asm_info(pnp_ctx *ctx, int64_t *full, int64_t *reused);
int pnp_matfree_info(pnp_ctx *ctx, int64_t *applies, int64_t *value_assemblies);

enum {
  PNP_CREATE_ABSORB_THIN_COLOR = 1
};
int pnp_set_create_option(int32_t option, int64_t value);
int pnp_get_create_option(int32_t option, int64_t *value);
int pnp_get_option(pnp_ctx *ctx, int32_t option, int64_t *value);

int pnp_linear_solve(pnp_ctx *ctx, const double *rhs, double *z, const pnp_solve_opts *opts,
                     pnp_solve_result *res);
int pnp_linear_solve_ex(pnp_ctx *ctx, const double *rhs, double *z, const pnp_solve_opts *opts,
                        pnp_solve_result *res, int32_t flags);

int pnp_solve_history(pnp_ctx *ctx, double *defects, int32_t cap, int32_t *n);

typedef struct {
  double reduction, abs_limit, min_linear_reduction;
  int32_t maxit, line_search_maxit;
  pnp_solve_opts linear;
} pnp_newton_opts;
typedef struct {
  int32_t converged, iterations, linear_iterations, status;
  double first_defect, defect, elapsed, assemble_seconds, solve_seconds;
  int32_t linear_fallbacks;
  int32_t precision_retries;
} pnp_newton_result;
int pnp_newton(pnp_ctx *ctx, double *u, const pnp_newton_opts *opts, pnp_newton_result *res);
int pnp_newton_history(pnp_ctx *ctx, int32_t *linear_iterations, double *defects, int32_t cap,
                       int32_t *nsteps);

int pnp_sync_vector(pnp_ctx *ctx, double *v, int32_t nfields);

int pnp_dot(pnp_ctx *ctx, const double *a, const double *b, int32_t nfields, int32_t flags,
            double *out);
int pnp_norm(pnp_ctx *ctx, const double *a, int32_t nfields, int32_t flags, double *out);

int pnp_initial_state(pnp_ctx *ctx, const double *phi_pb, double *x0);

int pnp_ion_flux(pnp_ctx *ctx, const double *x, int32_t nsurf, double *ip, double *im);

int pnp_state_set(pnp_ctx *ctx, const double *x);
int pnp_state_get(pnp_ctx *ctx, double *x);
int pnp_assemble_state(pnp_ctx *ctx, int32_t n);
int pnp_assemble_state_timed(pnp_ctx *ctx, int32_t n, double *ms);
int pnp_bicgstab_iterations(pnp_ctx *ctx, int32_t n, int32_t prec, pnp_solve_result *res);

typedef struct {
  double us_sell, us_tile, us_tile_sorted, us_random;
  int64_t slot_bytes;
  int64_t rows, rows_whole, tiles, elements;
} pnp_store_probe;
int pnp_probe_slot_stores(pnp_ctx *ctx, int32_t tile_elems, int32_t reps, pnp_store_probe *out);

int pnp_cache_scrub(pnp_ctx *ctx, int64_t bytes);

typedef struct {
  double assemble_ms, spmv_ms, prec_ms, blas_ms, halo_ms, allreduce_ms;
  int64_t assemble_launches, spmv_launches, prec_launches, blas_launches;
  double factor_ms;
  int64_t factor_launches;
} pnp_timers;
int pnp_timers_enable(pnp_ctx *ctx, int32_t on);
int pnp_timers_get(pnp_ctx *ctx, pnp_timers *t);
int pnp_timers_reset(pnp_ctx *ctx);


int pnp_setup_boundary(const pnp_mesh *mesh, const pnp_params *params, int32_t nfields,
                       int32_t field0, uint8_t *mask, double *load);
int pnp_setup_initial_state(const pnp_mesh *mesh, const pnp_params *params, const double *phi_pb,
                            double *x0);

typedef struct pnp_layout_buf pnp_layout_buf;
typedef struct {
  int32_t n_owned, n_ghost, ncolors, nchunks, nnbr, max_slots;
  int64_t nslots, nblocks;
  const int32_t *l2g;
  const int32_t *color_ptr;
  const int32_t *color_idx;
  const uint8_t *rowcolor;
  const int32_t *chunk_len;
  const int32_t *chunk_off;
  const int32_t *colidx;
  const uint64_t *rowmeta;
  const int32_t *nbr_ranks;
  const int32_t *recv_ptr;
  const int32_t *send_ptr;
  const int32_t *send_idx;
  int64_t color_conflicts;
} pnp_layout;
int pnp_layout_build(const pnp_mesh *mesh, int32_t rank, int32_t nranks, pnp_layout_buf **out);
int pnp_layout_view(const pnp_layout_buf *b, pnp_layout *view);
void pnp_layout_free(pnp_layout_buf *b);

#ifdef __cplusplus
}
#endif
#endif
```

Measured before the change: 51.84 billion assembled DOFs/s.

## Pipeline assembly tiles with LDS DMA prefetch of column indices and row flags

Adds a persistent, grid-strided variant of the constant-plane PNP Jacobian assembly kernel. Each wave uses global_load_lds to prefetch the next tile's column indices, row metadata and a new packed per-row flag byte into LDS, and reads chunk offsets through scalar constant loads. The residual tail now uses one flag byte per row in place of three dmask bytes and skips the cvec load when the row has no load term. The change trades simpler code for manual waitcnt handling and a host-built flag array, and it only runs when the pipe option and kconst path are enabled.

```diff
diff --git a/dune-pnp_amd/csrc/assemble.hip b/dune-pnp_amd/csrc/assemble.hip
--- a/dune-pnp_amd/csrc/assemble.hip
+++ b/dune-pnp_amd/csrc/assemble.hip
@@ -20,6 +20,23 @@
 #else
   store_vals_nt<NK, Q0>(vc + size_t(s) * NK * kRows, lane, Kc);
 #endif
+}
+
+template <int NF>
+__device__ __forceinline__ void residual_tail(const AsmArgs &a, int row, unsigned fl,
+                                              const double (&R)[NF]) {
+  double cv[NF];
+#pragma unroll
+  for (int f = 0; f < NF; f++) cv[f] = 0.0;
+  if (fl & kRowFlagLoad) {
+#pragma unroll
+    for (int f = 0; f < NF; f++) cv[f] = a.cvec[size_t(row) * NF + f];
+  }
+#pragma unroll
+  for (int f = 0; f < NF; f++) {
+    const double rv = R[f] + cv[f];
+    a.r[size_t(row) * NF + f] = ((fl >> f) & 1) ? 0.0 : rv;
+  }
 }
 
 template <int OP, int JAC, int MINW, int FANR>
@@ -147,12 +164,7 @@
     }
     store_block<OP>(vc, lane, 0, D);
   }
-#pragma unroll
-  for (int f = 0; f < NF; f++) {
-    const size_t q = size_t(row) * NF + f;
-    const double rv = R[f] + a.cvec[q];
-    a.r[q] = a.dmask[q] != 0 ? 0.0 : rv;
-  }
+  residual_tail<NF>(a, row, a.rowflag[row], R);
 }
 
 #ifndef ASM_SU
@@ -167,196 +179,273 @@
 constexpr int asm_kc() {
   return OP == OP_PNP;
 }
+constexpr int kPipeDw = 11;
+template <class P>
+__device__ __forceinline__ void lds_dma4(const P *src, uint32_t *dst_wave) {
+  __builtin_amdgcn_global_load_lds(
+      (const __attribute__((address_space(1))) void *)(src),
+      (__attribute__((address_space(3))) void *)(dst_wave), 4, 0, 0);
+}
+__device__ __forceinline__ int const_ld(const int *p, int i) {
+  return ((const __attribute__((address_space(4))) int *)(p))[i];
+}
+__device__ __forceinline__ int row_block_const(const DevLayout &L, int b, int nwg) {
+  return L.blkmap ? const_ld(L.blkmap, xcd_block(b, nwg, 1)) : xcd_block(b, nwg, L.xcd_remap);
+}
 template <int OP, int JAC, int MINW, int FANR, int SPLIT = FANR, int STAGE = 0, int LDSG = 0,
-          int KC = 0>
+          int KC = 0, int PIPE = 0>
 __global__ __launch_bounds__(256, MINW) void k_assemble_ga(DevLayout L, AsmArgs a) {
   using T = OpTraits<OP>;
   constexpr int NF = T::NF, NK = T::NK, NS = FANR;
   constexpr bool AUX0 = OP == OP_DIFF || OP == OP_DIFF_IE || OP == OP_POISSON;
   constexpr bool AUX1 = OP == OP_POISSON;
   constexpr int RW = asm_lds_rec<OP>();
+  static_assert(!PIPE || (JAC && FANR == 9 && !STAGE && !LDSG), "PIPE: the direct Jacobian walk");
   extern __shared__ double srec[];
-  const int blk = row_block(L, blockIdx.x, gridDim.x);
-  const int row0 = blk * blockDim.x + threadIdx.x;
-  const bool live = row0 < L.n_owned;
-  if (!LDSG && !live) return;
-  const int row = live ? row0 : 0;
-  const int chunk = row / kRows, lane = row % kRows;
-  const int off = L.chunk_off[chunk];
-  const uint64_t meta = L.rowmeta[row];
-  const int len = int(meta & 63);
-  const bool closed = (meta >> 6) & 1;
-  const unsigned brk = unsigned(meta >> 8);
-  double *__restrict__ vc = a.vals + size_t(off) * NK;
-
-  int cj[NS];
-  if constexpr (LDSG) {
-    const uint16_t *__restrict__ lix = L.lidx + off + lane;
-#pragma unroll
-    for (int k = 1; k < NS; k++) {
-      const int t = lix[(k < len ? k : 0) * kRows];
-      cj[k] = k < len ? t : 0;
-    }
-  } else {
-    const int *__restrict__ cix = L.colidx + off + lane;
-#pragma unroll
-    for (int k = 1; k < NS; k++) cj[k] = cix[(k < len ? k : 0) * kRows];
-  }
-  const double2 pi2 = reinterpret_cast<const double2 *>(L.xy)[row];
-  double ui[NF];
-  load_nf<NF>(a.x, size_t(row), ui);
-  double ai = 0, aq = 0;
-  if constexpr (AUX0) ai = a.aux0[row];
-  if constexpr (AUX1) aq = a.aux1[row];
-  if constexpr (OP == OP_PB) pb_fifth(ui[0], ai, aq);
-  if constexpr (LDSG) {
-    const int u0 = L.uptr[blk], cnt = L.uown[blk];
-    constexpr int kSU = ASM_SU;
-    int jj[kSU];
-#pragma unroll
-    for (int u = 0; u < kSU; u++) {
-      const int k = int(threadIdx.x) + u * 256;
-      jj[u] = k < cnt ? L.ulist[u0 + k] : -1;
-    }
-    double t[kSU][RW];
-#pragma unroll
-    for (int u = 0; u < kSU; u++)
-      if (jj[u] >= 0) {
-        const double2 p = reinterpret_cast<const double2 *>(L.xy)[jj[u]];
-        t[u][0] = p.x;
-        t[u][1] = p.y;
-        double uu[NF];
-        load_nf<NF>(a.x, size_t(jj[u]), uu);
-#pragma unroll
-        for (int f = 0; f < NF; f++) t[u][2 + f] = uu[f];
-        if constexpr (AUX0) t[u][2 + NF] = a.aux0[jj[u]];
-        if constexpr (AUX1) t[u][3 + NF] = a.aux1[jj[u]];
-      }
-#pragma unroll
-    for (int u = 0; u < kSU; u++)
-      if (jj[u] >= 0)
-#pragma unroll
-        for (int w = 0; w < RW; w++) srec[size_t(int(threadIdx.x) + u * 256) * RW + w] = t[u][w];
-    for (int k = int(threadIdx.x) + kSU * 256; k < cnt; k += blockDim.x) {
-      const int j = L.ulist[u0 + k];
-      const double2 p = reinterpret_cast<const double2 *>(L.xy)[j];
-      double u[NF];
-      load_nf<NF>(a.x, size_t(j), u);
-      double *r = srec + size_t(k) * RW;
-      r[0] = p.x;
-      r[1] = p.y;
-#pragma unroll
-      for (int f = 0; f < NF; f++) r[2 + f] = u[f];
-      if constexpr (AUX0) r[2 + NF] = a.aux0[j];
-      if constexpr (AUX1) r[3 + NF] = a.aux1[j];
-    }
-    __syncthreads();
-    if (!live) return;
-  }
-  double2 pn[NS];
-  double un[NS][NF], a0[NS], a1[NS];
-  auto gather = [&](int k) {
+  __shared__ uint32_t pfb[PIPE ? 4 * kPipeDw * kRows : 1];
+  const int ntiles = (L.n_owned + 255) / 256, G = gridDim.x;
+  const int wv = PIPE ? __builtin_amdgcn_readfirstlane(int(threadIdx.x) / kRows) : 0;
+  const int ln = int(threadIdx.x) % kRows;
+  uint32_t *const pw = pfb + (PIPE ? wv * kPipeDw * kRows : 0);
+  int tile = blockIdx.x, b0 = -1, b1 = -1, b2 = -1, o0 = 0, o1 = 0, c1 = 0;
+  auto tile_blk = [&](int t) { return t < ntiles ? row_block_const(L, t, ntiles) : -1; };
+  auto wave_chunk = [&](int b) {
+    return (b >= 0 && b * 256 + wv * kRows < L.n_owned) ? b * 4 + wv : -1;
+  };
+  auto prefetch = [&](int b, int off, int clen) {
+    if (wave_chunk(b) < 0) return;
+    const int r0 = b * 256 + wv * kRows;
+    const int *cix = L.colidx + off + ln;
+#pragma unroll
+    for (int k = 1; k < NS; k++)
+      lds_dma4(cix + (k < clen ? k : 0) * kRows, pw + (k - 1) * kRows);
+    const uint32_t *m =
+        reinterpret_cast<const uint32_t *>(L.rowmeta + min(r0 + ln, L.n_owned - 1));
+    lds_dma4(m, pw + 8 * kRows);
+    lds_dma4(m + 1, pw + 9 * kRows);
+    lds_dma4(reinterpret_cast<const uint32_t *>(a.rowflag + r0) + (ln >> 2), pw + 10 * kRows);
+  };
+  if constexpr (PIPE) {
+    if (tile >= ntiles) return;
+    b0 = tile_blk(tile);
+    b1 = tile_blk(tile + G);
+    b2 = tile_blk(tile + 2 * G);
+    int c0 = 0;
+    if (wave_chunk(b0) >= 0) {
+      o0 = const_ld(L.chunk_off, wave_chunk(b0));
+      c0 = const_ld(L.chunk_len, wave_chunk(b0));
+    }
+    if (wave_chunk(b1) >= 0) {
+      o1 = const_ld(L.chunk_off, wave_chunk(b1));
+      c1 = const_ld(L.chunk_len, wave_chunk(b1));
+    }
+    prefetch(b0, o0, c0);
+  }
+  int o2 = 0, c2 = 0, b3 = -1;
+  const auto advance = [&]() {
+    tile += G;
+    b0 = b1, o0 = o1;
+    b1 = b2, o1 = o2, c1 = c2;
+    b2 = b3;
+    return b0 >= 0;
+  };
+  do {
+    const int blk = PIPE ? b0 : row_block(L, blockIdx.x, gridDim.x);
+    const int row0 = blk * blockDim.x + threadIdx.x;
+    const bool live = row0 < L.n_owned;
+    if (!PIPE && !LDSG && !live) return;
+    const int row = live ? row0 : 0;
+    const int chunk = row / kRows, lane = row % kRows;
+    int cj[NS];
+    uint64_t meta_pf = 0;
+    unsigned fl_pf = 0;
+    if constexpr (PIPE) {
+      asm volatile("s_waitcnt vmcnt(0)" ::: "memory");
+#pragma unroll
+      for (int k = 1; k < NS; k++) cj[k] = int(pw[(k - 1) * kRows + ln]);
+      meta_pf = uint64_t(pw[8 * kRows + ln]) | (uint64_t(pw[9 * kRows + ln]) << 32);
+      fl_pf = (pw[10 * kRows + ln] >> (8 * (ln & 3))) & 0xffu;
+      asm volatile("s_waitcnt lgkmcnt(0)" ::: "memory");
+      prefetch(b1, o1, c1);
+      o2 = c2 = 0;
+      if (wave_chunk(b2) >= 0) {
+        o2 = const_ld(L.chunk_off, wave_chunk(b2));
+        c2 = const_ld(L.chunk_len, wave_chunk(b2));
+      }
+      b3 = tile_blk(tile + 3 * G);
+      if (!live) continue;
+    }
+    const int off = PIPE ? o0 : L.chunk_off[chunk];
+    const uint64_t meta = PIPE ? meta_pf : L.rowmeta[row];
+    const int len = int(meta & 63);
+    const bool closed = (meta >> 6) & 1;
+    const unsigned brk = unsigned(meta >> 8);
+    double *__restrict__ vc = a.vals + size_t(off) * NK;
+
+    if constexpr (PIPE) {
+    } else if constexpr (LDSG) {
+      const uint16_t *__restrict__ lix = L.lidx + off + lane;
+#pragma unroll
+      for (int k = 1; k < NS; k++) {
+        const int t = lix[(k < len ? k : 0) * kRows];
+        cj[k] = k < len ? t : 0;
+      }
+    } else {
+      const int *__restrict__ cix = L.colidx + off + lane;
+#pragma unroll
+      for (int k = 1; k < NS; k++) cj[k] = cix[(k < len ? k : 0) * kRows];
+    }
+    const double2 pi2 = reinterpret_cast<const double2 *>(L.xy)[row];
+    double ui[NF];
+    load_nf<NF>(a.x, size_t(row), ui);
+    double ai = 0, aq = 0;
+    if constexpr (AUX0) ai = a.aux0[row];
+    if constexpr (AUX1) aq = a.aux1[row];
+    if constexpr (OP == OP_PB) pb_fifth(ui[0], ai, aq);
     if constexpr (LDSG) {
-      const double *r = srec + size_t(cj[k]) * RW;
-      pn[k] = make_double2(r[0], r[1]);
-#pragma unroll
-      for (int f = 0; f < NF; f++) un[k][f] = r[2 + f];
-      a0[k] = AUX0 ? r[2 + NF] : 0.0;
-      a1[k] = AUX1 ? r[3 + NF] : 0.0;
-    } else {
-      pn[k] = reinterpret_cast<const double2 *>(L.xy)[cj[k]];
-      load_nf<NF>(a.x, size_t(cj[k]), un[k]);
-      a0[k] = AUX0 ? a.aux0[cj[k]] : 0.0;
-      a1[k] = AUX1 ? a.aux1[cj[k]] : 0.0;
-    }
-  };
-#pragma unroll
-  for (int k = 1; k < SPLIT; k++) gather(k);
-  if constexpr (OP == OP_PB) pb_fifth(un[1][0], a0[1], a1[1]);
-
-  double R[NF], D[NK], P[NK], F[NK];
-#pragma unroll
-  for (int f = 0; f < NF; f++) R[f] = 0;
-#pragma unroll
-  for (int v = 0; v < NK; v++) D[v] = P[v] = F[v] = 0;
-  constexpr int NSTG = (STAGE && JAC && SPLIT < NS && SPLIT > 3) ? SPLIT - 3 : 0;
-  __shared__ double stg[NSTG > 0 ? NSTG * NK * 256 : 1];
-  unsigned staged = 0;
-  auto put = [&](int s, const double *Kc) {
-    if (NSTG > 0 && s <= NSTG) {
-#pragma unroll
-      for (int v = 0; v < NK; v++) stg[((s - 1) * NK + v) * 256 + threadIdx.x] = Kc[v];
-      staged |= 1u << s;
-    } else {
-      store_block<OP, KC>(vc, lane, s, Kc);
-    }
-  };
-#pragma unroll
-  for (int s = 1; s < NS; s++) {
-    if (SPLIT < NS && s == (SPLIT > 2 ? SPLIT - 2 : 1)) {
-#pragma unroll
-      for (int k = SPLIT; k < NS; k++) gather(k);
-      if constexpr (NSTG > 0) {
-#pragma unroll
-        for (int q = 1; q <= NSTG; q++)
-          if ((staged >> q) & 1) {
-            double K[NK];
-#pragma unroll
-            for (int v = 0; v < NK; v++) K[v] = stg[((q - 1) * NK + v) * 256 + threadIdx.x];
-            store_block<OP, KC>(vc, lane, q, K);
+      const int u0 = L.uptr[blk], cnt = L.uown[blk];
+      constexpr int kSU = ASM_SU;
+      int jj[kSU];
+#pragma unroll
+      for (int u = 0; u < kSU; u++) {
+        const int k = int(threadIdx.x) + u * 256;
+        jj[u] = k < cnt ? L.ulist[u0 + k] : -1;
+      }
+      double t[kSU][RW];
+#pragma unroll
+      for (int u = 0; u < kSU; u++)
+        if (jj[u] >= 0) {
+          const double2 p = reinterpret_cast<const double2 *>(L.xy)[jj[u]];
+          t[u][0] = p.x;
+          t[u][1] = p.y;
+          double uu[NF];
+          load_nf<NF>(a.x, size_t(jj[u]), uu);
+#pragma unroll
+          for (int f = 0; f < NF; f++) t[u][2 + f] = uu[f];
+          if constexpr (AUX0) t[u][2 + NF] = a.aux0[jj[u]];
+          if constexpr (AUX1) t[u][3 + NF] = a.aux1[jj[u]];
+        }
+#pragma unroll
+      for (int u = 0; u < kSU; u++)
+        if (jj[u] >= 0)
+#pragma unroll
+          for (int w = 0; w < RW; w++) srec[size_t(int(threadIdx.x) + u * 256) * RW + w] = t[u][w];
+      for (int k = int(threadIdx.x) + kSU * 256; k < cnt; k += blockDim.x) {
+        const int j = L.ulist[u0 + k];
+        const double2 p = reinterpret_cast<const double2 *>(L.xy)[j];
+        double u[NF];
+        load_nf<NF>(a.x, size_t(j), u);
+        double *r = srec + size_t(k) * RW;
+        r[0] = p.x;
+        r[1] = p.y;
+#pragma unroll
+        for (int f = 0; f < NF; f++) r[2 + f] = u[f];
+        if constexpr (AUX0) r[2 + NF] = a.aux0[j];
+        if constexpr (AUX1) r[3 + NF] = a.aux1[j];
+      }
+      __syncthreads();
+      if (!live) return;
+    }
+    double2 pn[NS];
+    double un[NS][NF], a0[NS], a1[NS];
+    auto gather = [&](int k) {
+      if constexpr (LDSG) {
+        const double *r = srec + size_t(cj[k]) * RW;
+        pn[k] = make_double2(r[0], r[1]);
+#pragma unroll
+        for (int f = 0; f < NF; f++) un[k][f] = r[2 + f];
+        a0[k] = AUX0 ? r[2 + NF] : 0.0;
+        a1[k] = AUX1 ? r[3 + NF] : 0.0;
+      } else {
+        pn[k] = reinterpret_cast<const double2 *>(L.xy)[cj[k]];
+        load_nf<NF>(a.x, size_t(cj[k]), un[k]);
+        a0[k] = AUX0 ? a.aux0[cj[k]] : 0.0;
+        a1[k] = AUX1 ? a.aux1[cj[k]] : 0.0;
+      }
+    };
+#pragma unroll
+    for (int k = 1; k < SPLIT; k++) gather(k);
+    if constexpr (OP == OP_PB) pb_fifth(un[1][0], a0[1], a1[1]);
+
+    double R[NF], D[NK], P[NK], F[NK];
+#pragma unroll
+    for (int f = 0; f < NF; f++) R[f] = 0;
+#pragma unroll
+    for (int v = 0; v < NK; v++) D[v] = P[v] = F[v] = 0;
+    constexpr int NSTG = (STAGE && JAC && SPLIT < NS && SPLIT > 3) ? SPLIT - 3 : 0;
+    __shared__ double stg[NSTG > 0 ? NSTG * NK * 256 : 1];
+    unsigned staged = 0;
+    auto put = [&](int s, const double *Kc) {
+      if (NSTG > 0 && s <= NSTG) {
+#pragma unroll
+        for (int v = 0; v < NK; v++) stg[((s - 1) * NK + v) * 256 + threadIdx.x] = Kc[v];
+        staged |= 1u << s;
+      } else {
+        store_block<OP, KC>(vc, lane, s, Kc);
+      }
+    };
+#pragma unroll
+    for (int s = 1; s < NS; s++) {
+      if (SPLIT < NS && s == (SPLIT > 2 ? SPLIT - 2 : 1)) {
+#pragma unroll
+        for (int k = SPLIT; k < NS; k++) gather(k);
+        if constexpr (NSTG > 0) {
+#pragma unroll
+          for (int q = 1; q <= NSTG; q++)
+            if ((staged >> q) & 1) {
+              double K[NK];
+#pragma unroll
+              for (int v = 0; v < NK; v++) K[v] = stg[((q - 1) * NK + v) * 256 + threadIdx.x];
+              store_block<OP, KC>(vc, lane, q, K);
+            }
+        }
+      }
+      if (s < len) {
+        const bool has_next = s + 1 < len;
+        const int sn = (s + 1 < NS) ? s + 1 : 1;
+        const bool elem = (has_next || closed) && !((brk >> s) & 1);
+        if constexpr (OP == OP_PB)
+          if (has_next) pb_fifth(un[sn][0], a0[sn], a1[sn]);
+        if (elem) {
+          const double2 pt = has_next ? pn[sn] : pn[1];
+          double ut[NF];
+#pragma unroll
+          for (int f = 0; f < NF; f++) ut[f] = has_next ? un[sn][f] : un[1][f];
+          const double at0 = has_next ? a0[sn] : a0[1], at1 = has_next ? a1[sn] : a1[1];
+          Geo G;
+          geometry(pi2.x, pi2.y, pn[s].x, pn[s].y, pt.x, pt.y, G);
+          double Ct[NK];
+#pragma unroll
+          for (int v = 0; v < NK; v++) Ct[v] = 0;
+          element<OP, JAC, KC>(a, G, pi2.y, pn[s].y, pt.y, ui, un[s], ut, ai, a0[s], at0, aq,
+                               a1[s], at1, R, D, P, Ct);
+          if constexpr (JAC) {
+            if (s == 1 && closed) {
+#pragma unroll
+              for (int v = 0; v < NK; v++) F[v] = P[v];
+            } else {
+              put(s, P);
+            }
+#pragma unroll
+            for (int v = 0; v < NK; v++) P[v] = Ct[v];
           }
-      }
-    }
-    if (s < len) {
-      const bool has_next = s + 1 < len;
-      const int sn = (s + 1 < NS) ? s + 1 : 1;
-      const bool elem = (has_next || closed) && !((brk >> s) & 1);
-      if constexpr (OP == OP_PB)
-        if (has_next) pb_fifth(un[sn][0], a0[sn], a1[sn]);
-      if (elem) {
-        const double2 pt = has_next ? pn[sn] : pn[1];
-        double ut[NF];
-#pragma unroll
-        for (int f = 0; f < NF; f++) ut[f] = has_next ? un[sn][f] : un[1][f];
-        const double at0 = has_next ? a0[sn] : a0[1], at1 = has_next ? a1[sn] : a1[1];
-        Geo G;
-        geometry(pi2.x, pi2.y, pn[s].x, pn[s].y, pt.x, pt.y, G);
-        double Ct[NK];
-#pragma unroll
-        for (int v = 0; v < NK; v++) Ct[v] = 0;
-        element<OP, JAC, KC>(a, G, pi2.y, pn[s].y, pt.y, ui, un[s], ut, ai, a0[s], at0, aq,
-                             a1[s], at1, R, D, P, Ct);
-        if constexpr (JAC) {
-          if (s == 1 && closed) {
-#pragma unroll
-            for (int v = 0; v < NK; v++) F[v] = P[v];
-          } else {
-            put(s, P);
-          }
-#pragma unroll
-          for (int v = 0; v < NK; v++) P[v] = Ct[v];
+        } else if constexpr (JAC) {
+          put(s, P);
+#pragma unroll
+          for (int v = 0; v < NK; v++) P[v] = 0;
         }
-      } else if constexpr (JAC) {
-        put(s, P);
-#pragma unroll
-        for (int v = 0; v < NK; v++) P[v] = 0;
-      }
-    }
-  }
-  if constexpr (JAC) {
-    if (closed) {
-#pragma unroll
-      for (int v = 0; v < NK; v++) F[v] += P[v];
-      store_block<OP, KC>(vc, lane, 1, F);
-    }
-    store_block<OP, KC>(vc, lane, 0, D);
-  }
-#pragma unroll
-  for (int f = 0; f < NF; f++) {
-    const size_t q = size_t(row) * NF + f;
-    const double rv = R[f] + a.cvec[q];
-    a.r[q] = a.dmask[q] != 0 ? 0.0 : rv;
-  }
+      }
+    }
+    if constexpr (JAC) {
+      if (closed) {
+#pragma unroll
+        for (int v = 0; v < NK; v++) F[v] += P[v];
+        store_block<OP, KC>(vc, lane, 1, F);
+      }
+      store_block<OP, KC>(vc, lane, 0, D);
+    }
+    residual_tail<NF>(a, row, PIPE ? fl_pf : unsigned(a.rowflag[row]), R);
+  } while (PIPE && advance());
 }
 
 template <int OP>
@@ -446,8 +535,35 @@
   return hipGetLastError();
 }
 
+constexpr bool kAsmPipeDefault = false;
+
+template <int OP>
+static int launch_pipe(const DevLayout &L, const AsmArgs &a, int cap, hipStream_t s, hipEvent_t t0,
+                       hipEvent_t t1) {
+  if constexpr (asm_kc<OP>()) {
+    const auto kern = k_assemble_ga<OP, 1, 3, 9, 6, 0, 0, 1, 1>;
+    static const int resident = [&] {
+      int dev = 0, cus = 0, per_cu = 0;
+      if (hipGetDevice(&dev) != hipSuccess ||
+          hipDeviceGetAttribute(&cus, hipDeviceAttributeMultiprocessorCount, dev) != hipSuccess ||
+          hipOccupancyMaxActiveBlocksPerMultiprocessor(&per_cu, kern, 256, 0) != hipSuccess)
+        return 0;
+      return per_cu * cus;
+    }();
+    const int ntiles = (L.n_owned + 255) / 256;
+    int g = resident >= 8 ? resident / 8 * 8 : 8;
+    if (g > ntiles) g = ntiles;
+    if (cap > 0 && g > cap) g = cap;
+    hipExtLaunchKernelGGL(kern, dim3(g), dim3(256), 0, s, t0, t1, 0, L, a);
+    return 1;
+  } else {
+    return 0;
+  }
+}
+
 hipError_t launch_assemble(const DevLayout &L, const AsmArgs &a, hipStream_t s, hipEvent_t t0,
-                           hipEvent_t t1) {
+                           hipEvent_t t1, int *pipelined) {
+  if (pipelined) *pipelined = 0;
   if (L.n_owned == 0) return hipSuccess;
   dim3 grid((L.n_owned + 255) / 256), block(256);
   static const int waves = [] {
@@ -476,6 +592,15 @@
            (lds_env < 0 && (size_t(L.n_owned) * 7 * size_t(nk) * 8 > (size_t(512) << 20) ||
                             (cold_hint && a.cold)));
   };
+  static const bool pipe_on = [] {
+    const char *e = getenv("PNP_ASM_PIPE");
+    return e ? atoi(e) != 0 : kAsmPipeDefault;
+  }();
+  static const int pipe_cap = [] {
+    const char *e = getenv("PNP_ASM_PIPE_GRID");
+    return (e && atoi(e) >= 1) ? atoi(e) : 0;
+  }();
+  int piped = 0;
 #define PNP_ASM_CASE(OPK)                                                          \
   case OPK:                                                                        \
     if (!fanr && a.jac)                                                            \
@@ -501,6 +626,8 @@
              size_t(L.unmax) * asm_lds_rec<OPK>() * 8 <= 53 * 1024)                    \
       hipExtLaunchKernelGGL((k_assemble_ga<OPK, 1, 3, 9, 6, 0, 1, asm_kc<OPK>()>), grid,  \
                          block, size_t(L.unmax) * asm_lds_rec<OPK>() * 8, s, t0, t1, 0, L, a); \
+    else if (ga == 4 && fanr == 9 && asm_kc<OPK>() && a.kconst && pipe_on)         \
+      piped = launch_pipe<OPK>(L, a, pipe_cap, s, t0, t1);                         \
     else if (ga == 4 && fanr == 9 && asm_kc<OPK>() && a.kconst)                    \
       hipExtLaunchKernelGGL((k_assemble_ga<OPK, 1, 3, 9, 6, 0, 0, asm_kc<OPK>()>), grid,  \
                          block, 0, s, t0, t1, 0, L, a);                             \
@@ -532,6 +659,7 @@
     return hipErrorInvalidValue;
   }
 #undef PNP_ASM_CASE
+  if (pipelined) *pipelined = piped;
   return hipGetLastError();
 }
 
diff --git a/dune-pnp_amd/csrc/ctx.cc b/dune-pnp_amd/csrc/ctx.cc
--- a/dune-pnp_amd/csrc/ctx.cc
+++ b/dune-pnp_amd/csrc/ctx.cc
@@ -249,6 +249,8 @@
   std::vector<int> fseg_group;
   DBuf<double> fluxout, fluxx, fluxred;
   DBuf<uint8_t> dmask;
+  DBuf<uint8_t> rowflag;
+  std::vector<uint8_t> hrowflag;
   DBuf<double> cvec, aux0, aux1;
   bool assembled = false;
   bool after_solve = false;
@@ -265,7 +267,7 @@
     return (e && std::atoi(e) == 0) ? 0 : 1;
   }();
   bool vals_const_valid = false;
-  long long asm_full = 0, asm_reused = 0;
+  long long asm_full = 0, asm_reused = 0, asm_piped = 0;
   bool asm_kconst() const {
     return asm_reuse_opt && vals_const_valid && degree == 1 && !fd_mode && kind == PNP_OP_PNP;
   }
@@ -772,10 +774,11 @@
       t0 = tb(T_ASM);
     }
     hipError_t e;
+    int piped = 0;
     if (degree > 1)
       e = pnp::launch_pk_assemble(dl, aa, pkd, jac ? (fd_mode ? 2 : 1) : 0, stream);
     else
-      e = pnp::launch_assemble(dl, aa, stream, t1 ? t0 : nullptr, t1);
+      e = pnp::launch_assemble(dl, aa, stream, t1 ? t0 : nullptr, t1, &piped);
     if (e == hipSuccess && jac && fd_mode && degree == 1)
       e = pnp::launch_fd_jacobian(dl, aa, nf, pat, fd_ne, fd_etri.p, fd_rptr.p, fd_cdata.p,
                                   fd_jel.p, stream);
@@ -784,6 +787,7 @@
       return hipfail(e, "assemble");
     }
     if (jac && !mf) asm_wrote(aa.kconst != 0, degree == 1 && !fd_mode);
+    asm_piped += piped;
     if (t1) {
       ev_pending[T_ASM].push_back({t0, t1});
       t_n[T_ASM]++;
@@ -832,12 +836,14 @@
     fa.cold = after_solve ? 1 : 0;
     fa.kconst = asm_kconst() ? 1 : 0;
     hipEvent_t t0 = tb(T_ASM);
-    e = pnp::launch_assemble(dl, fa, stream);
+    int piped = 0;
+    e = pnp::launch_assemble(dl, fa, stream, nullptr, nullptr, &piped);
     if (e != hipSuccess) {
       vals_const_valid = false;
       return hipfail(e, "assemble at the linearisation point");
     }
     asm_wrote(fa.kconst != 0, true);
+    asm_piped += piped;
     te(T_ASM, t0);
     vals_stale = false;
     value_assemblies++;
@@ -3315,6 +3321,7 @@
                "partials2")) ||
       (rc = al(c->S, 2, "scalars")) || (rc = al(c->redmw, pnp::kRedMwDoubles, "reduce ticket")) ||
       (rc = al(c->dmask, 3 * size_t(L.n_owned), "dmask")) ||
+      (rc = al(c->rowflag, size_t(L.nchunks + 1) * pnp::kRows, "row flags")) ||
       (rc = al(c->cvec, 3 * size_t(L.n_owned), "cvec")) || (rc = al(c->aux0, nloc, "aux0")) ||
       (rc = al(c->aux1, nloc, "aux1"))) {
     g_err = c->err;
@@ -3519,6 +3526,25 @@
       if (a->c_extra) lload[size_t(i) * nf + f] += a->c_extra[size_t(f) * m.nv + L.l2g[i]];
     }
   CK(hipMemcpy(c->dmask.p, lmask.data(), lmask.size(), hipMemcpyHostToDevice), "dmask");
+  {
+    std::vector<uint8_t> flag(c->rowflag.n, 0);
+    for (int i = 0; i < L.n_owned; i++) {
+      unsigned fl = ie ? pnp::kRowFlagLoad : 0;
+      for (int f = 0; f < nf; f++) {
+        if (lmask[size_t(i) * nf + f]) fl |= 1u << f;
+        uint64_t bits;
+        std::memcpy(&bits, &lload[size_t(i) * nf + f], sizeof bits);
+        if (bits) fl |= pnp::kRowFlagLoad;
+        if (a->c_extra) {
+          std::memcpy(&bits, &a->c_extra[size_t(f) * m.nv + L.l2g[i]], sizeof bits);
+          if (bits) fl |= pnp::kRowFlagLoad;
+        }
+      }
+      flag[i] = uint8_t(fl);
+    }
+    CK(hipMemcpy(c->rowflag.p, flag.data(), flag.size(), hipMemcpyHostToDevice), "row flags");
+    c->hrowflag.assign(flag.begin(), flag.begin() + L.n_owned);
+  }
   c->seq_op_valid = false;
   c->seq_dt = a->dt;
   c->seq_z = a->z;
@@ -3576,6 +3602,7 @@
   aa.aux1 = c->aux1.p;
   aa.cvec = c->cvec.p;
   aa.dmask = c->dmask.p;
+  aa.rowflag = c->rowflag.p;
   aa.vals = c->vals.p;
   return PNP_OK;
 }
@@ -4043,10 +4070,20 @@
   return PNP_OK;
 }
 
-extern "C" int pnp_asm_info(pnp_ctx *c, int64_t *full, int64_t *reused) {
+extern "C" int pnp_asm_row_flags(pnp_ctx *c, uint8_t *flags) {
+  if (!c || !flags) return PNP_E_ARG;
+  if (c->kind < 0) return c->fail(PNP_E_STATE, "no operator set (pnp_set_operator)");
+  if (c->degree > 1) return c->fail(PNP_E_STATE, "row flags: P1 contexts only");
+  std::memset(flags, 0xff, size_t(c->mesh.nv));
+  for (int i = 0; i < c->L.n_owned; i++) flags[c->L.l2g[i]] = c->hrowflag[i];
+  return PNP_OK;
+}
+
+extern "C" int pnp_asm_info(pnp_ctx *c, int64_t *full, int64_t *reused, int64_t *pipelined) {
   if (!c) return PNP_E_ARG;
   if (full) *full = c->asm_full;
   if (reused) *reused = c->asm_reused;
+  if (pipelined) *pipelined = c->asm_piped;
   return PNP_OK;
 }
 
diff --git a/dune-pnp_amd/csrc/kernels.h b/dune-pnp_amd/csrc/kernels.h
--- a/dune-pnp_amd/csrc/kernels.h
+++ b/dune-pnp_amd/csrc/kernels.h
@@ -209,6 +209,8 @@
   return dm;
 }
 
+constexpr unsigned kRowFlagMask = 7, kRowFlagLoad = 8;
+
 struct AsmArgs {
   int kind;
   int jac;
@@ -219,6 +221,7 @@
   const double *aux1;
   const double *cvec;
   const uint8_t *dmask;
+  const uint8_t *rowflag;
   double *r;
   double *vals;
   int cold;
@@ -238,7 +241,8 @@
 };
 
 hipError_t launch_assemble(const DevLayout &L, const AsmArgs &a, hipStream_t s,
-                           hipEvent_t t0 = nullptr, hipEvent_t t1 = nullptr);
+                           hipEvent_t t0 = nullptr, hipEvent_t t1 = nullptr,
+                           int *pipelined = nullptr);
 hipError_t launch_ion_flux(int ns, const int4 *seg, const double *xy, const double *x, int cyl,
                            double pi, double *out, hipStream_t s);
 hipError_t launch_mass_apply(const DevLayout &L, int kind, double tau, double pi, int cylindrical,
diff --git a/dune-pnp_amd/python/pnp_amd/__init__.py b/dune-pnp_amd/python/pnp_amd/__init__.py
--- a/dune-pnp_amd/python/pnp_amd/__init__.py
+++ b/dune-pnp_amd/python/pnp_amd/__init__.py
@@ -21,6 +21,8 @@
  OPT_GRAPH, OPT_SEQ_ORDER, OPT_ILU_FLOW, OPT_NAT_FLOW, OPT_ILU_RETRY,
  OPT_GMRES_RESTART, OPT_MATRIX_FREE, OPT_ASM_REUSE_CONST) = (1, 2, 3, 4, 5, 6, 7, 8, 9, 10, 11,
                                                              12, 13)
+ASM_PIPE_ENV, ASM_PIPE_GRID_ENV = "PNP_ASM_PIPE", "PNP_ASM_PIPE_GRID"
+ROW_FLAG_LOAD = 8
 DEVICE_PTRS, JAC_FD = 1, 2
 CREATE_ABSORB_THIN_COLOR = 1
 PREC_BY_NAME = {"none": PREC_NONE, "nonprec": PREC_NONE, "ssor": PREC_SSOR, "ilu0": PREC_ILU0,
@@ -729,9 +731,14 @@
         return {"applies": a.value, "value_assemblies": v.value}
 
     def asm_info(self):
-        f, r = C.c_int64(), C.c_int64()
-        self._ck(lib().pnp_asm_info(self.h, C.byref(f), C.byref(r)))
-        return {"full": f.value, "reused": r.value}
+        f, r, p = C.c_int64(), C.c_int64(), C.c_int64()
+        self._ck(lib().pnp_asm_info(self.h, C.byref(f), C.byref(r), C.byref(p)))
+        return {"full": f.value, "reused": r.value, "pipelined": p.value}
+
+    def asm_row_flags(self):
+        out = np.zeros(self.mesh.nv, dtype=np.uint8)
+        self._ck(lib().pnp_asm_row_flags(self.h, out.ctypes.data_as(C.c_void_p)))
+        return out
 
     def probe_slot_stores(self, tile_elems=256, reps=20):
         o = _StoreProbe()
diff --git a/include/pnp_capi.h b/include/pnp_capi.h
--- a/include/pnp_capi.h
+++ b/include/pnp_capi.h
@@ -221,7 +221,9 @@
   PNP_OPT_ASM_REUSE_CONST = 13
 };
 int pnp_set_option(pnp_ctx *ctx, int32_t option, int64_t value);
-int pnp_asm_info(pnp_ctx *ctx, int64_t *full, int64_t *reused);
+int pnp_asm_info(pnp_ctx *ctx, int64_t *full, int64_t *reused, int64_t *pipelined);
+#define PNP_ROW_FLAG_LOAD 8
+int pnp_asm_row_flags(pnp_ctx *ctx, uint8_t *flags);
 int pnp_matfree_info(pnp_ctx *ctx, int64_t *applies, int64_t *value_assemblies);
 
 enum {
```

After: 54.39 billion assembled DOFs/s (median of 6 runs). 1.05x the previous value.
